# hongfz16/AvatarCLIP

Hardware: AMD Instinct MI355X
Metric: rays_per_sec_512x512_64spp_clip_guided_train_iter (higher is better)
Workload: dtype f16 (forward) / bf16 (gradient sweeps) MFMA operands, fp32 accumulate

## Files before the change

avatarclip_amd/csrc/avc_bwd_body.h:

```cpp
#pragma once
#include "avc_mlp.h"
constexpr int BWD_G = 4;
constexpr int BWD_WPB = 8;

template <typename P> __device__ __forceinline__ P launder(P p) {
  asm volatile("" : "+s"(p));
  return p;
}
__device__ __forceinline__ float second_term(float gbar_h, float g_a, float s) {
  const float r = s > 1e-30f ? __builtin_amdgcn_rcpf(s) : 0.f;
  return gbar_h * g_a * (AVC_BETA * (1.f - s) * r);
}
struct PF3 { h8 h0, h1; b8 b0, b1; h8 g0, g1; };

struct BwdArgs {
  PointSrc ps;
  long npts;
  const b8* Wb0;
  const float* T0;
  const float* d_sdf;
  const float* d_normal;
  const float* d_rgb;
  const float* rgb_fwd;
  const char* fpanels;
  char* gpanels;
  const unsigned short* masks;
  float* colsum;
};

#define AVC_CS_DUMMY 64
template <class N> struct ColSum {
  static constexpr int SLOT_FLOATS = PanelLayout<N>::CS_FLOATS + AVC_CS_DUMMY;
  static constexpr int LDS_BYTES = BWD_WPB * SLOT_FLOATS * 4;
};
typedef AVC_LDS float* cs_slot_t;
__device__ __forceinline__ float quad_xor1(float x) {
  return __builtin_bit_cast(float, __builtin_amdgcn_update_dpp(0, __builtin_bit_cast(int, x), 0xB1, 0xf, 0xf, true));
}
__device__ __forceinline__ float quad_xor2(float x) {
  return __builtin_bit_cast(float, __builtin_amdgcn_update_dpp(0, __builtin_bit_cast(int, x), 0x4E, 0xf, 0xf, true));
}
template <int NV>
__device__ __forceinline__ float transpose_sum(const float (&v)[NV], int lane) {
  static_assert(NV == 8 || NV == 16, "8 or 16 values per lane");
  float w[NV / 2];
  const bool b0 = lane & 1, b1 = lane & 2, b2 = lane & 4, b3 = lane & 8;
#pragma unroll
  for (int k = 0; k < NV / 2; ++k) w[k] = (b0 ? v[2 * k + 1] : v[2 * k]) + quad_xor1(b0 ? v[2 * k] : v[2 * k + 1]);
  float x[NV / 4];
#pragma unroll
  for (int k = 0; k < NV / 4; ++k) x[k] = (b1 ? w[2 * k + 1] : w[2 * k]) + quad_xor2(b1 ? w[2 * k] : w[2 * k + 1]);
  float y[NV / 8];
#pragma unroll
  for (int k = 0; k < NV / 8; ++k) y[k] = (b2 ? x[2 * k + 1] : x[2 * k]) + __shfl_xor(b2 ? x[2 * k] : x[2 * k + 1], 4);
  float z;
  if constexpr (NV == 16) z = (b3 ? y[1] : y[0]) + __shfl_xor(b3 ? y[0] : y[1], 8);
  else z = y[0] + __shfl_xor(y[0], 8);
  return z + __shfl_xor(z, 16);
}
template <class N, int NV>
__device__ __forceinline__ void col_sums(cs_slot_t slot, int lane, int base, const float (&v)[NV]) {
  const float total = transpose_sum<NV>(v, lane);
  const bool writer = (lane & 31) < NV;
  cs_slot_t dst = writer ? slot + base + (lane & (NV - 1)) : slot + PanelLayout<N>::CS_FLOATS + (lane & 63);
  *dst = *dst + total;
}
template <class N>
__device__ __forceinline__ cs_slot_t cs_init(char* lds_base, int wv, int lane) {
  cs_slot_t slot = (cs_slot_t)lds_base + wv * ColSum<N>::SLOT_FLOATS;
  for (int k = lane; k < ColSum<N>::SLOT_FLOATS; k += 64) slot[k] = 0.f;
  return slot;
}
template <class N>
__device__ __forceinline__ void cs_flush(cs_slot_t slot, float* out, long row, int lane) {
  asm volatile("s_waitcnt lgkmcnt(0)" ::: "memory");
  for (int k = lane; k < PanelLayout<N>::CS_FLOATS; k += 64) out[row * PanelLayout<N>::CS_FLOATS + k] = slot[k];
}

template <class N> struct BlkIn { b8 dof; unsigned m1[N::HT], m2[N::HT]; float dn[3], dsdf; };
template <class N>
__device__ __forceinline__ void load_blk_in(const BwdArgs& a, long blk, long nblk, int lane, BlkIn<N>& bi) {
  typedef PanelLayout<N> L;
  const int h = lane >> 5, p = lane & 31;
  long i = blk * 32 + p;
  const float vmask = i < a.npts ? 1.f : 0.f;
  if (i >= a.npts) i = a.npts - 1;
  bi.dof = zero_frag<b8>();
#pragma unroll
  for (int r = 0; r < 4; ++r) {
    const int ch = h ? 4 + r : r;
    const float c = (ch < 6) ? a.rgb_fwd[6 * i + (ch < 6 ? ch : 0)] : 0.f;
    const float dr = (ch < 6) ? a.d_rgb[6 * i + (ch < 6 ? ch : 0)] * vmask : 0.f;
    bi.dof[r] = (__bf16)(dr * c * (1.f - c));
  }
  const AVC_GLOBAL unsigned short* mk = as_global(a.masks) + (blk < nblk ? blk : nblk) * (long)L::MASK_U16 + lane;
#pragma unroll
  for (int t = 0; t < N::HT; ++t) {
    bi.m1[t] = mk[t * 64];
    bi.m2[t] = (N::NCMID == 1) ? mk[(N::HT + t) * 64] : 0u;
  }
#pragma unroll
  for (int c = 0; c < 3; ++c) bi.dn[c] = a.d_normal[3 * i + c] * vmask;
  bi.dsdf = a.d_sdf[i] * vmask;
}

template <class N>
__device__ __forceinline__ void bwd_sweeps(StageT<BWD_G>& sg, const BwdArgs& a, lds_tab_t Tl, long blk0, long nblk, int lane0,
                                           int wv, cs_slot_t cs, BlkIn<N>& bi, long blk0_next) {
  typedef PanelLayout<N> L;
  constexpr AvcOffsets o = Off<N>::value;
  const PointSrc& ps = a.ps;
  const long npts = a.npts;
  const b8* Wb = launder(a.Wb0);
  lds_tab_t T = Tl;
  asm volatile("" : "+s"(T));
  int lane = lane0;
  asm volatile("" : "+v"(lane));
  const int h = lane >> 5, p = lane & 31;
  sg.lane = lane;
  const long blk = blk0 + wv;
  const long bsel = blk < nblk ? blk : nblk;
  const PanelPtr ftiles = panel_ptr(const_cast<char*>(a.fpanels) + bsel * (long)L::P_TILES * 2048, lane);
  const PanelPtr tiles = panel_ptr(a.gpanels + bsel * (long)L::G_TILES * 2048, lane);
  long i = blk * 32 + p;
  const bool valid = i < npts;
  if (!valid) i = npts - 1;
  const float vmask = valid ? 1.f : 0.f;
  float x[3];
  fetch_point(ps, i, x);
  float nbar[3];
  float dsdf_in;
  {
    b8 dof[1];
    dof[0] = bi.dof;
    tile_store<false>(tiles, L::G_DO, dof[0], zero_frag<b8>());
    unsigned m1[N::HT], m2[N::HT];
#pragma unroll
    for (int t = 0; t < N::HT; ++t) { m1[t] = bi.m1[t]; m2[t] = bi.m2[t]; }
    const float dn_in[3] = {bi.dn[0], bi.dn[1], bi.dn[2]};
    dsdf_in = bi.dsdf;
#define AVC_RELU_BWD(OUT, MSK, PT)                                                                         \
  AVC_EPI(const unsigned bits = MSK[t];                                                                      \
          _Pragma("unroll") for (int j = 0; j < 8; ++j) {                                                    \
            OUT[2 * t][j] = (__bf16)(((bits >> relu_mask_bit(j)) & 1u) ? acc[j] : 0.f);                      \
            OUT[2 * t + 1][j] = (__bf16)(((bits >> relu_mask_bit(8 + j)) & 1u) ? acc[8 + j] : 0.f); }        \
          pin2(OUT[2 * t], OUT[2 * t + 1]);                                                                  \
          tile_store<false>(tiles, (PT) + t, OUT[2 * t], OUT[2 * t + 1]);)
    b8 dl[N::HK];
    b8 d1[N::HK];
    if constexpr (N::NCMID == 1) {
      layer_s1<b8, 1, N::HT>(sg, Wb, o.v[OFF_CHT], nxt<N, OFF_CM0T>(sg, Wb, o), dof, AVC_RELU_BWD(dl, m2, L::G_D2));
      layer_s1<b8, N::HK, N::HT>(sg, Wb, o.v[OFF_CM0T], nxt<N, OFF_C0T>(sg, Wb, o), dl, AVC_RELU_BWD(d1, m1, L::G_D1));
    } else {
      layer_s1<b8, 1, N::HT>(sg, Wb, o.v[OFF_CHT], nxt<N, OFF_C0T>(sg, Wb, o), dof, AVC_RELU_BWD(d1, m1, L::G_D1));
    }
    float dn_acc[3] = {0.f, 0.f, 0.f};
    layer_s1<b8, N::HK, N::HT + 1>(sg, Wb, o.v[OFF_C0T], nxt<N, OFF_W0G>(sg, Wb, o), d1, AVC_EPI(
      if (t < N::HT) {
        b8 f0, f1;
        _Pragma("unroll") for (int j = 0; j < 8; ++j) { f0[j] = (__bf16)acc[j]; f1[j] = (__bf16)acc[8 + j]; }
        pin2(f0, f1);
        tile_store<true>(tiles, L::G_DFEAT + (t < N::HT ? t : 0), f0, f1);
      } else {
        dn_acc[0] = acc[3]; dn_acc[1] = acc[0]; dn_acc[2] = acc[1];
      }
    ));
    {
      const float a3 = dn_acc[0], a0 = dn_acc[1], a1 = dn_acc[2];
      const float o3 = __shfl_xor(a3, 32), o0 = __shfl_xor(a0, 32), o1 = __shfl_xor(a1, 32);
      nbar[0] = valid ? dn_in[0] + (h ? o3 : a3) : 0.f;
      nbar[1] = valid ? dn_in[1] + (h ? a0 : o0) : 0.f;
      nbar[2] = valid ? dn_in[2] + (h ? a1 : o1) : 0.f;
    }
  }
  const float dsdf = dsdf_in;
  const float dsdfS = dsdf * AVC_S;
  {
    b8 fs = zero_frag<b8>();
    if (h == 0) {
      fs[0] = (__bf16)dsdf;
      fs[1] = (__bf16)(dsdf - (float)fs[0]);
    }
    tile_store<false>(tiles, L::G_SDF, fs, zero_frag<b8>());
  }
  b8 gbs[N::SK];
  b8 dfeat[N::HK];
  auto load_dfeat = [&]() __attribute__((always_inline)) {
#pragma unroll
    for (int t = 0; t < N::HT; ++t) {
      const FragPair<b8> d = tile_load<true, b8>(tiles, L::G_DFEAT + t);
      dfeat[2 * t] = d.a0;
      dfeat[2 * t + 1] = d.a1;
    }
  };
  {
    b8 gb0[3];
    {
      PE pe4;
      pe_compute(x, h, pe4);
      float g0[24];
#pragma unroll
      for (int q = 0; q < 24; ++q) {
        g0[q] = pe4.d[q] * nbar[q % 3];
        gb0[q >> 3][q & 7] = (__bf16)g0[q];
      }
#pragma unroll
      for (int s = 0; s < 3; ++s) {
        float v[8];
#pragma unroll
        for (int j = 0; j < 8; ++j) v[j] = g0[8 * s + j];
        col_sums<N, 8>(cs, lane, N::ST * 32 + (s * 2 + h) * 8, v);
      }
    }
    tile_store<false>(tiles, L::G_GB0, gb0[0], gb0[1]);
    tile_store<false>(tiles, L::G_GB0 + 1, gb0[2], zero_frag<b8>());
#define AVC_E_LOADH(PH) tile_load<false, h8>(ftiles, (PH) + t)
#define AVC_SECOND(OUT, PH, PT)                                                                              \
  AVC_PRE(return AVC_E_LOADH(PH);),                                                                          \
  AVC_EPID(FragPair<h8>, _Pragma("unroll") for (int j = 0; j < 8; ++j) {                                     \
            OUT[2 * t][j] = (__bf16)(acc[j] * sig_from_h((float)d.a0[j]));                                   \
            OUT[2 * t + 1][j] = (__bf16)(acc[8 + j] * sig_from_h((float)d.a1[j])); }                         \
          pin2(OUT[2 * t], OUT[2 * t + 1]);                                                                  \
          tile_store<true>(tiles, (PT) + t, OUT[2 * t], OUT[2 * t + 1]);)
#define AVC_SECOND_S(OUT, PH)                                                                                \
  AVC_PRE(return AVC_E_LOADH(PH);),                                                                          \
  AVC_EPID(FragPair<h8>, float v[16];                                                                        \
          _Pragma("unroll") for (int j = 0; j < 8; ++j) {                                                    \
            v[j] = acc[j] * sig_from_h((float)d.a0[j]);                                                      \
            v[8 + j] = acc[8 + j] * sig_from_h((float)d.a1[j]);                                              \
            OUT[2 * t][j] = (__bf16)v[j];                                                                    \
            OUT[2 * t + 1][j] = (__bf16)v[8 + j]; }                                                          \
          pin2(OUT[2 * t], OUT[2 * t + 1]);                                                                  \
          col_sums<N, 16>(cs, lane, (t * 2 + h) * 16, v);)
    b8 gb1[N::HK];
    layer_sq1<b8, 3, N::HT>(sg, Wb, o.v[OFF_W0G], nxt<N, OFF_WM0>(sg, Wb, o), gb0, AVC_SECOND(gb1, L::P_H1, L::G_GBH1));
    b8 gbm[N::HK];
    layer_sq1<b8, N::HK, N::HT>(sg, Wb, o.v[OFF_WM0], nxt<N, (N::NMID == 2 ? OFF_WM1 : OFF_WS)>(sg, Wb, o), gb1,
                                AVC_SECOND(gbm, L::P_HM, L::G_GBHM));
    b8 gbm1[N::HK];
    if constexpr (N::NMID == 2)
      layer_sq1<b8, N::HK, N::HT>(sg, Wb, o.v[OFF_WM1], nxt<N, OFF_WS>(sg, Wb, o), gbm,
                                  AVC_SECOND(gbm1, L::P_HM + N::HT, L::G_GBHM + N::HT));
    layer_sq1<b8, N::HK, N::ST>(sg, Wb, o.v[OFF_WS], nxt<N, OFF_WLT>(sg, Wb, o), (N::NMID == 2 ? gbm1 : gbm), AVC_SECOND_S(gbs, L::P_HS));
  }
  {
    b8 as_[N::SK];
    load_dfeat();
#define AVC_F_LOADB(PB) tile_load<true, b8>(tiles, (PB) + t)
#define AVC_LOAD3(PH, PB, PG)                                                                               \
  AVC_PRE(PF3 d; { const FragPair<h8> a_ = tile_load<true, h8>(ftiles, (PH) + t); d.h0 = a_.a0; d.h1 = a_.a1; } \
          { const FragPair<b8> a_ = AVC_F_LOADB(PB); d.b0 = a_.a0; d.b1 = a_.a1; } \
          { const FragPair<h8> a_ = tile_load<true, h8>(ftiles, (PG) + t); d.g0 = a_.a0; d.g1 = a_.a1; } return d;)
#define AVC_LOAD3_S(PH, PG)                                                                                 \
  AVC_PRE(PF3 d; { const FragPair<h8> a_ = tile_load<true, h8>(ftiles, (PH) + t); d.h0 = a_.a0; d.h1 = a_.a1; } \
          d.b0 = gbs[2 * t]; d.b1 = gbs[2 * t + 1];                                                          \
          { const FragPair<h8> a_ = tile_load<true, h8>(ftiles, (PG) + t); d.g0 = a_.a0; d.g1 = a_.a1; } return d;)
    layer_sq1<b8, N::HK, N::ST>(sg, Wb, o.v[OFF_WLT], nxt<N, OFF_WST>(sg, Wb, o), dfeat,
      AVC_LOAD3_S(L::P_HS, L::P_GAS), AVC_EPID(PF3,
      float wa[16];
      load16(T + o.v[OFF_WL0_ACC], t, h, wa);
      _Pragma("unroll") for (int j = 0; j < 8; ++j) {
        const float s0 = sig_from_h((float)d.h0[j]), s1 = sig_from_h((float)d.h1[j]);
        as_[2 * t][j] = (__bf16)(second_term((float)d.b0[j], (float)d.g0[j], s0) + (acc[j] + wa[j] * dsdfS) * s0);
        as_[2 * t + 1][j] = (__bf16)(second_term((float)d.b1[j], (float)d.g1[j], s1) + (acc[8 + j] + wa[8 + j] * dsdfS) * s1);
      }
      pin2(as_[2 * t], as_[2 * t + 1]);
      tile_store<false>(tiles, L::G_ABS + t, as_[2 * t], as_[2 * t + 1]);
    ));
#define AVC_REVERSE(OUT, PH, PB, PG, PT)                                                                    \
  AVC_LOAD3(PH, PB, PG),                                                                                     \
  AVC_EPID(PF3, _Pragma("unroll") for (int j = 0; j < 8; ++j) {                                              \
            const float s0 = sig_from_h((float)d.h0[j]), s1 = sig_from_h((float)d.h1[j]);                    \
            OUT[2 * t][j] = (__bf16)(second_term((float)d.b0[j], (float)d.g0[j], s0) + acc[j] * s0);         \
            OUT[2 * t + 1][j] = (__bf16)(second_term((float)d.b1[j], (float)d.g1[j], s1) + acc[8 + j] * s1); } \
          pin2(OUT[2 * t], OUT[2 * t + 1]);                                                                  \
          tile_store<false>(tiles, (PT) + t, OUT[2 * t], OUT[2 * t + 1]);)
    b8 am[N::HK];
    b8 am0[N::HK];
    const Next first = nxt<N, OFF_CHT>(sg, a.Wb0, o);
#define AVC_F_LASTHOOK AVC_HOOK(load_blk_in<N>(a, blk0_next + wv, nblk, lane, bi);)
    constexpr int TOP = (N::NMID - 1) * N::HT;
    layer_sq1<b8, N::SK, N::HT>(sg, Wb, o.v[OFF_WST], nxt<N, (N::NMID == 2 ? OFF_WM1T : OFF_WM0T)>(sg, Wb, o), as_,
                               AVC_REVERSE(am, L::P_HM + TOP, L::G_GBHM + TOP, L::P_GAM + TOP, L::G_ABM + TOP));
    if constexpr (N::NMID == 2)
      layer_sq1<b8, N::HK, N::HT>(sg, Wb, o.v[OFF_WM1T], nxt<N, OFF_WM0T>(sg, Wb, o), am,
                                 AVC_REVERSE(am0, L::P_HM, L::G_GBHM, L::P_GAM, L::G_ABM));
    layer_sq1<b8, N::HK, N::HT>(sg, Wb, o.v[OFF_WM0T], first, (N::NMID == 2 ? am0 : am),
                               AVC_REVERSE((N::NMID == 2 ? am : am0), L::P_H1, L::G_GBH1, L::P_GA1, L::G_AB1), AVC_F_LASTHOOK);
  }
#undef AVC_RELU_BWD
#undef AVC_SECOND
#undef AVC_LOAD3
#undef AVC_LOAD3_S
#undef AVC_F_LOADB
#undef AVC_E_LOADH
#undef AVC_SECOND_S
#undef AVC_F_LASTHOOK
#undef AVC_REVERSE
}
```

avatarclip_amd/csrc/avc_mlp.h:

```cpp
#pragma once
#include "avc_common.h"
#include "avc_stage.h"

template <int H_, int NMID_, int NCMID_>
struct NetT {
  static constexpr int H = H_;
  static constexpr int NMID = NMID_;
  static constexpr int NCMID = NCMID_;
  static constexpr int HT = H / 32;
  static constexpr int HK = H / 16;
  static constexpr int SKIP = H - 39;
  static constexpr int ST = (SKIP + 31) / 32;
  static constexpr int SK = 2 * ST;
  static_assert(H % 32 == 0 && SKIP > 0 && ST <= HT, "hidden width: a multiple of 32 above 39");
};
typedef NetT<256, 2, 1> NetFull;
typedef NetT<128, 1, 0> NetSmall;
typedef NetT<128, 2, 1> NetH128Deep;
typedef NetT<256, 1, 0> NetH256Shallow;
typedef NetT<64, 2, 1> NetH64Deep;
typedef NetT<64, 1, 0> NetH64Shallow;
template <class N> struct NetTag { typedef N type; };
template <typename R, typename F>
static inline R with_net(int net, R unknown, F&& f) {
  switch (net) {
    case 0: return f(NetTag<NetFull>{});
    case 1: return f(NetTag<NetSmall>{});
    case 2: return f(NetTag<NetH128Deep>{});
    case 3: return f(NetTag<NetH256Shallow>{});
    case 4: return f(NetTag<NetH64Deep>{});
    case 5: return f(NetTag<NetH64Shallow>{});
    default: return unknown;
  }
}
template <typename F>
static inline void for_each_net(F&& f) {
  for (int id = 0; with_net(id, false, [&](auto tag) { f(tag); return true; }); ++id) {}
}
#include "avc_offsets_gen.h"
template <class N> static inline bool offsets_match(const int* offs) {
  for (int k = 0; k < OFF_COUNT; ++k)
    if (offs[k] != Off<N>::value.v[k]) return false;
  return true;
}

struct PointSrc {
  const float* pts;
  const float* rays_o;
  const float* rays_d;
  const float* z;
  int S;
  int ldz;
  int midpoint;
  float sample_dist;
};

__device__ __forceinline__ void fetch_point(const PointSrc& ps, long i, float (&x)[3]) {
  if (ps.pts) {
    x[0] = ps.pts[3 * i]; x[1] = ps.pts[3 * i + 1]; x[2] = ps.pts[3 * i + 2];
    return;
  }
  const long ray = i / ps.S;
  const int s = (int)(i - ray * ps.S);
  const float* zr = ps.z + ray * ps.ldz;
  float t = zr[s];
  if (ps.midpoint) {
    const float dist = (s + 1 < ps.S) ? (zr[s + 1] - t) : ps.sample_dist;
    t = t + dist * 0.5f;
  }
#pragma unroll
  for (int c = 0; c < 3; ++c) x[c] = ps.rays_o[3 * ray + c] + ps.rays_d[3 * ray + c] * t;
}

template <typename V, int KS>
__device__ __forceinline__ const V* tptr(const V* blob, int off, int t, int lane) {
  return blob + (off >> 3) + (long)(t * KS) * 64 + lane;
}


template <class N, int OFF> struct TileInfo;
#define AVC_TI(OFF, KS_, NT_) template <class N> struct TileInfo<N, OFF> { static constexpr int KS = KS_, NT = NT_; };
AVC_TI(OFF_W0, 3, N::HT)          AVC_TI(OFF_WM0, N::HK, N::HT)   AVC_TI(OFF_WM1, N::HK, N::HT)  AVC_TI(OFF_WS, N::HK, N::ST)
AVC_TI(OFF_WL, N::SK + 3, N::HT)  AVC_TI(OFF_W0T, N::HK, 2)       AVC_TI(OFF_WM0T, N::HK, N::HT) AVC_TI(OFF_WM1T, N::HK, N::HT)
AVC_TI(OFF_WST, N::SK, N::HT)     AVC_TI(OFF_WLT, N::HK, N::ST)   AVC_TI(OFF_C0, N::HK + 1, N::HT) AVC_TI(OFF_CM0, N::HK, N::HT)
AVC_TI(OFF_CH, N::HK, 1)          AVC_TI(OFF_C0T, N::HK, N::HT + 1) AVC_TI(OFF_CM0T, N::HK, N::HT) AVC_TI(OFF_CHT, 1, N::HT)
AVC_TI(OFF_W0G, 3, N::HT)

template <class N, int OFF, class ST>
__device__ __forceinline__ Next nxt(const ST&, const void* blob, const AvcOffsets& o) {
  typedef TileInfo<N, OFF> TI;
  Next n;
  n.ptr = reinterpret_cast<const char*>(blob) + (long)o.v[OFF] * 2;
  constexpr int G = ST::template group<TI::KS>();
  static_assert(G >= 1 && G <= ST::G && TI::KS * 1024 * G <= ST::BUF_BYTES && TI::NT >= 1, "staging group of this layer");
  n.chunks = TI::KS * (TI::NT < G ? TI::NT : G);
  return n;
}
__device__ __forceinline__ Next no_next() { Next n; n.ptr = nullptr; n.chunks = 0; return n; }

#define AVC_SYNC() __syncthreads()
#define AVC_EPI(...) [&](int t, const facc& acc) __attribute__((always_inline)) { __VA_ARGS__ }
struct NoHook { __device__ __forceinline__ void operator()() const {} };
#define AVC_HOOK(...) [&]() __attribute__((always_inline)) { __VA_ARGS__ }
#define AVC_HOOKG(...) [&](int grp_, int ngrp_) __attribute__((always_inline)) { __VA_ARGS__ }
template <typename Hook>
__device__ __forceinline__ void hook_call(Hook&& hook, int g) {
  if constexpr (!std::is_invocable_v<Hook, int, int>) { if (g == 0) hook(); }
}
template <typename Hook>
__device__ __forceinline__ void hook_tile(Hook&& hook, int t, int nt) {
  if constexpr (std::is_invocable_v<Hook, int, int>) hook(t, nt);
}

#define AVC_PRE(...) [&](int t) __attribute__((always_inline)) { __VA_ARGS__ }
#define AVC_EPID(DT, ...) [&](int t, const facc& acc, const DT& d) __attribute__((always_inline)) { __VA_ARGS__ }
struct NoPre { __host__ __device__ __forceinline__ int operator()(int) const { return 0; } };
template <bool PAIRED, int KS, int NT, class ST, typename V, typename Mma, typename Pre, typename Epi, typename Hook>
__device__ __forceinline__ void layer_walk(ST& st, const V* __restrict__ blob, int offw, const Next& after, Mma&& mma, Pre&& pre,
                                           Epi&& epi, Hook&& hook) {
  constexpr int G = ST::template group<KS>();
  constexpr int NG = (NT + G - 1) / G;
  constexpr bool LOADS = !std::is_same_v<std::decay_t<Pre>, NoPre>;
  typedef std::invoke_result_t<Pre&, int> D;
  auto finish = [&](int t, const facc& acc, const D& d) __attribute__((always_inline)) {
    if constexpr (LOADS) epi(t, acc, d);
    else epi(t, acc);
  };
  facc prev0, prev1;
  D d0{}, d1{};
  int tp = -1, np = 0;
#pragma unroll
  for (int g = 0; g < NG; ++g) {
    AVC_SYNC();
    if (g + 1 < NG) {
      Next n;
      n.ptr = blob + (offw >> 3) + (long)((g + 1) * G * KS) * 64;
      n.chunks = KS * ((NT - (g + 1) * G) < G ? (NT - (g + 1) * G) : G);
      stage_issue(st, n, st.par ^ 1);
    } else {
      stage_issue(st, after, st.par ^ 1);
    }
    hook_call(hook, g);
#pragma unroll
    for (int j = 0; j < G; j += (PAIRED ? 2 : 1)) {
      const int t = g * G + j;
      if (t < NT) {
        const bool two = PAIRED && (j + 1 < G) && (t + 1 < NT);
        hook_tile(hook, t, NT);
        if (two) hook_tile(hook, t + 1, NT);
        if (LOADS && np > 0) {
          d0 = pre(tp);
          if (np > 1) d1 = pre(tp + 1);
          __builtin_amdgcn_sched_barrier(0);
        }
        facc a0, a1;
        mma(j, t, two, a0, a1);
        if (np > 0) {
          finish(tp, prev0, d0);
          if (np > 1) finish(tp + 1, prev1, d1);
          if (two) { interleave_mfma_valu<KS>(); interleave_mfma_valu<KS>(); } else interleave_mfma_valu<KS>();
        }
        prev0 = a0;
        if (two) prev1 = a1;
        tp = t; np = two ? 2 : 1;
        __builtin_amdgcn_sched_barrier(0);
      }
    }
    st.par ^= 1;
  }
  if constexpr (LOADS) {
    d0 = pre(tp);
    if (np > 1) d1 = pre(tp + 1);
  }
  finish(tp, prev0, d0);
  if (np > 1) finish(tp + 1, prev1, d1);
  __builtin_amdgcn_sched_barrier(0);
}
template <bool PAIRED, typename V, int KS, int NT, class ST, typename Pre, typename Epi, typename Hook, class Bias>
__device__ __forceinline__ void layer_sp(ST& st, const V* __restrict__ blob, int offw, const Next& after, const V (&in)[KS],
                                         Pre&& pre, Epi&& epi, Hook&& hook, const Bias& bias) {
  layer_walk<PAIRED, KS, NT>(st, blob, offw, after, [&](int j, int t, bool two, facc& a0, facc& a1) __attribute__((always_inline)) {
    if (two) tile_mma_pair<V, KS>(st, j, in, a0, a1, bias, t);
    else a0 = tile_mma<V, KS>(st, j, in, bias, t);
  }, pre, epi, hook);
}
template <typename V, int KS, int NT, class ST, typename Epi, typename Hook = NoHook, class Bias = NoBias>
__device__ __forceinline__ void layer_s(ST& st, const V* __restrict__ blob, int offw, const Next& after, const V (&in)[KS],
                                        Epi&& epi, Hook&& hook = NoHook{}, const Bias& bias = NoBias{}) {
  layer_sp<true, V, KS, NT>(st, blob, offw, after, in, NoPre{}, epi, hook, bias);
}
template <typename V, int KS, int NT, class ST, typename Epi, typename Hook = NoHook, class Bias = NoBias>
__device__ __forceinline__ void layer_s1(ST& st, const V* __restrict__ blob, int offw, const Next& after, const V (&in)[KS],
                                         Epi&& epi, Hook&& hook = NoHook{}, const Bias& bias = NoBias{}) {
  layer_sp<false, V, KS, NT>(st, blob, offw, after, in, NoPre{}, epi, hook, bias);
}
template <typename V, int KS, int NT, class ST, typename Pre, typename Epi, typename Hook = NoHook>
__device__ __forceinline__ void layer_sq(ST& st, const V* __restrict__ blob, int offw, const Next& after, const V (&in)[KS],
                                         Pre&& pre, Epi&& epi, Hook&& hook = NoHook{}) {
  layer_sp<true, V, KS, NT>(st, blob, offw, after, in, pre, epi, hook, NoBias{});
}
template <typename V, int KS, int NT, class ST, typename Pre, typename Epi, typename Hook = NoHook>
__device__ __forceinline__ void layer_sq1(ST& st, const V* __restrict__ blob, int offw, const Next& after, const V (&in)[KS],
                                          Pre&& pre, Epi&& epi, Hook&& hook = NoHook{}) {
  layer_sp<false, V, KS, NT>(st, blob, offw, after, in, pre, epi, hook, NoBias{});
}
template <typename V, int KA, int KB, int NT, class ST, typename Epi, typename Hook = NoHook, class Bias = NoBias>
__device__ __forceinline__ void layer2_s(ST& st, const V* __restrict__ blob, int offw, const Next& after, const V (&ina)[KA],
                                         const V (&inb)[KB], Epi&& epi, Hook&& hook = NoHook{}, const Bias& bias = NoBias{}) {
  layer_walk<true, KA + KB, NT>(st, blob, offw, after, [&](int j, int t, bool two, facc& a0, facc& a1) __attribute__((always_inline)) {
    if (two) tile_mma2_pair<V, KA, KB>(st, j, ina, inb, a0, a1, bias, t);
    else a0 = tile_mma2<V, KA, KB>(st, j, ina, inb, bias, t);
  }, NoPre{}, epi, hook);
}

template <class N>
struct PanelLayout {
  static constexpr int HT = N::HT, ST = N::ST, NM = N::NMID, NC = N::NCMID;
  static constexpr int P_H1 = 0;
  static constexpr int P_HM = P_H1 + HT;
  static constexpr int P_HS = P_HM + NM * HT;
  static constexpr int P_H0 = P_HS + ST;
  static constexpr int P_GA1 = P_H0 + 2;
  static constexpr int P_GAM = P_GA1 + HT;
  static constexpr int P_GAS = P_GAM + NM * HT;
  static constexpr int P_FEAT = P_GAS + ST;
  static constexpr int P_XN = P_FEAT + HT;
  static constexpr int P_R1 = P_XN + 1;
  static constexpr int P_R2 = P_R1 + HT;
  static constexpr int P_TILES = P_R2 + NC * HT;
  static constexpr int G_GBH1 = 0;
  static constexpr int G_GBHM = G_GBH1 + HT;
  static constexpr int G_GB0 = G_GBHM + NM * HT;
  static constexpr int G_AB1 = G_GB0 + 2;
  static constexpr int G_ABM = G_AB1 + HT;
  static constexpr int G_ABS = G_ABM + NM * HT;
  static constexpr int G_DFEAT = G_ABS + ST;
  static constexpr int G_SDF = G_DFEAT + HT;
  static constexpr int G_D1 = G_SDF + 1;
  static constexpr int G_D2 = G_D1 + HT;
  static constexpr int G_DO = G_D2 + NC * HT;
  static constexpr int G_TILES = G_DO + 1;
  static constexpr int MASK_U16 = 2 * HT * 64;
  static constexpr int CS_FLOATS = ST * 32 + 48;
};
template <class N>
struct ScratchLayout {
  static constexpr int HT = N::HT, NM = N::NMID;
  static constexpr int P_H1 = 0, P_HM = HT, P_FEAT = HT + NM * HT, P_TILES = P_FEAT + HT;
  static constexpr int P_H0 = 0, P_HS = 0, P_GA1 = 0, P_GAM = 0, P_GAS = 0, P_XN = 0, P_R1 = 0, P_R2 = 0;
};

struct PanelPtr {
  AVC_GLOBAL char* ub;
  unsigned off;
};
__device__ __forceinline__ PanelPtr panel_ptr(char* base, int lane) {
  const unsigned long long v = (unsigned long long)base;
  const unsigned lo = __builtin_amdgcn_readfirstlane((unsigned)v), hi = __builtin_amdgcn_readfirstlane((unsigned)(v >> 32));
  PanelPtr p;
  p.ub = (AVC_GLOBAL char*)(((unsigned long long)hi << 32) | lo);
  p.off = (unsigned)lane * 16u;
  return p;
}
template <typename V> __device__ __forceinline__ AVC_GLOBAL V* tile_addr(const PanelPtr& pp, int tile) {
  AVC_GLOBAL char* tb = pp.ub + (long)tile * 2048;
  asm("" : "+s"(tb));
  return (AVC_GLOBAL V*)(tb + pp.off);
}
template <typename V>
__device__ __forceinline__ V zero_frag() {
  V z;
#pragma unroll
  for (int j = 0; j < 8; ++j) z[j] = (typename MF<V>::S)0.f;
  return z;
}
template <bool KEEP, typename V>
__device__ __forceinline__ void tile_store(const PanelPtr& pp, int tile, const V& f0, const V& f1) {
  AVC_GLOBAL V* p = tile_addr<V>(pp, tile);
  if (KEEP) {
    p[0] = f0;
    p[64] = f1;
  } else {
    AVC_NT_STORE(f0, &p[0]);
    AVC_NT_STORE(f1, &p[64]);
  }
}
template <bool KEEP, int NT, typename V, int KS>
__device__ __forceinline__ void tiles_store(const PanelPtr& pp, int tile0, const V (&f)[KS]) {
#pragma unroll
  for (int t = 0; t < NT; ++t) tile_store<KEEP>(pp, tile0 + t, f[2 * t], f[2 * t + 1]);
}
template <bool KEEP, int NT, typename V, int KS>
__device__ __forceinline__ void tiles_store_part(const PanelPtr& pp, int tile0, const V (&f)[KS], int g, int ng) {
#pragma unroll
  for (int t = 0; t < NT; ++t)
    if (t * ng / NT == g) tile_store<KEEP>(pp, tile0 + t, f[2 * t], f[2 * t + 1]);
}
template <typename V> struct FragPair { V a0, a1; };
template <bool NT, typename V>
__device__ __forceinline__ FragPair<V> tile_load(const PanelPtr& pp, int tile) {
  const AVC_GLOBAL V* p = tile_addr<V>(pp, tile);
  FragPair<V> d;
  if (NT) { d.a0 = AVC_NT_LOAD(&p[0]); d.a1 = AVC_NT_LOAD(&p[64]); }
  else { d.a0 = p[0]; d.a1 = p[64]; }
  return d;
}

#define AVC_SDF_ACT(OUT)                                                                      \
  AVC_EPI(float a[16];                                                                        \
          softplus2_tile(acc, a);                                                             \
          acc_to_frags(a, OUT[2 * t], OUT[2 * t + 1]);)
template <class N, class ST, typename TP>
__device__ __forceinline__ float sdf_only(ST& sg, const h8* __restrict__ Wf, TP T, const AvcOffsets& o,
                                          int h, const float (&x)[3]) {
  PE pe;
  pe_compute(x, h, pe);
  float part = 0.f;
  {
    const auto wpe = T + o.v[OFF_WL0_PE] + h * 24;
#pragma unroll
    for (int q = 0; q < 24; ++q) part += wpe[q] * pe.v[q];
    asm volatile("" : "+v"(part));
  }
  h8 hlast[N::HK];
  {
    h8 h1[N::HK];
    {
      h8 pef[3];
      pe_to_frags_f16(pe, x, h, pef);
      layer_s1<h8, 3, N::HT>(sg, Wf, o.v[OFF_W0], nxt<N, OFF_WM0>(sg, Wf, o), pef, AVC_SDF_ACT(h1),
                             NoHook{}, TabBias{T + o.v[OFF_B0], h});
    }
    h8 hm0[N::HK];
    layer_s1<h8, N::HK, N::HT>(sg, Wf, o.v[OFF_WM0], nxt<N, (N::NMID == 2 ? OFF_WM1 : OFF_WS)>(sg, Wf, o), h1,
                               AVC_SDF_ACT((N::NMID == 2 ? hm0 : hlast)), NoHook{}, TabBias{T + o.v[OFF_BM0], h});
    if constexpr (N::NMID == 2)
      layer_s1<h8, N::HK, N::HT>(sg, Wf, o.v[OFF_WM1], nxt<N, OFF_WS>(sg, Wf, o), hm0, AVC_SDF_ACT(hlast),
                                 NoHook{}, TabBias{T + o.v[OFF_BM1], h});
  }
  layer_s1<h8, N::HK, N::ST>(sg, Wf, o.v[OFF_WS], no_next(), hlast, AVC_EPI(
    float w[16];
    load16(T + o.v[OFF_WL0_ACC], t, h, w);
    _Pragma("unroll") for (int r = 0; r < 16; ++r) part += w[r] * softplus2(acc[r]);
  ), NoHook{}, TabBias{T + o.v[OFF_BS], h});
  return xhalf_sum(part) + T[o.v[OFF_BL0]];
}
#undef AVC_SDF_ACT
```

avatarclip_amd/csrc/avc_mlp_bwd.hip:

```cpp
#include "avc_bwd_body.h"
#include "../../include/avc.h"

template <class N>
__global__ __launch_bounds__(64 * BWD_WPB) void mlp_bwd_kernel(BwdArgs a) {
  extern __shared__ __attribute__((aligned(16))) char lds[];
  typedef StageT<BWD_G> ST;
  constexpr AvcOffsets o = Off<N>::value;
  static_assert(BWD_WPB >= 4 && BWD_WPB % 4 == 0, "stage_issue's turns need a multiple of 4 wavefronts per workgroup");
  const int lane0 = threadIdx.x & 63;
  const int wv = threadIdx.x >> 6;
  const long nblk = (a.npts + 31) >> 5;
  ST sg = stage_init<BWD_G>(lds);
  stage_issue(sg, nxt<N, OFF_CHT>(sg, a.Wb0, o), 0);
  const lds_tab_t Tl = tab_to_lds(lds + ST::LDS_BYTES, a.T0, o.v[OFF_TAB_END]);
  const cs_slot_t cs = cs_init<N>(lds + ST::LDS_BYTES + AVC_TAB_LDS_BYTES, wv, lane0);
  __syncthreads();
  BlkIn<N> bi;
  load_blk_in<N>(a, (long)blockIdx.x * BWD_WPB + wv, nblk, lane0, bi);
  for (long blk0 = (long)blockIdx.x * BWD_WPB; blk0 < nblk; blk0 += (long)gridDim.x * BWD_WPB)
    bwd_sweeps<N>(sg, a, Tl, blk0, nblk, lane0, wv, cs, bi, blk0 + (long)gridDim.x * BWD_WPB);
  cs_flush<N>(cs, a.colsum, (long)blockIdx.x * BWD_WPB + wv, lane0);
}

extern "C" int avc_bwd_colsum_floats(int net) {
  return with_net<int>(net, 0, [](auto tag) -> int { return PanelLayout<typename decltype(tag)::type>::CS_FLOATS; });
}
extern "C" long avc_bwd_colsum_rows(long npts, long max_waves) {
  const long nblk = (npts + 31) / 32;
  long ngroups = (nblk + BWD_WPB - 1) / BWD_WPB, maxg = max_waves / BWD_WPB;
  if (maxg < 1) maxg = 1;
  long grid = ngroups < maxg ? ngroups : maxg;
  if (grid < 1) grid = 1;
  return grid * BWD_WPB;
}

extern "C" int avc_render_points_bwd(int net, const float* pts, const float* rays_o, const float* rays_d, const float* z,
                                     int S, int ldz, float sample_dist, long npts, const void* wbf16, const float* tab,
                                     const int* offs, const float* d_sdf, const float* d_normal, const float* d_rgb,
                                     const float* rgb_fwd, const void* fpanels, void* gpanels, const void* masks, float* colsum,
                                     long max_waves, void* stream) {
  if (npts <= 0) return 0;
  if (!fpanels || !gpanels || !masks || !rgb_fwd || !colsum) { avc_set_error("avc_render_points_bwd: fpanels / gpanels / masks / rgb_fwd / colsum == NULL"); return 1; }
  const int bad = with_net<int>(net, 2, [&](auto tag) -> int { return offsets_match<typename decltype(tag)::type>(offs) ? 0 : 1; });
  if (bad == 1) { avc_set_error("packed-blob offsets differ from the compiled-in table (regenerate csrc/avc_offsets_gen.h)"); return 1; }
  if (bad == 2) { avc_set_error("unknown net id"); return 1; }
  PointSrc ps{pts, rays_o, rays_d, z, S, ldz, pts ? 0 : 1, sample_dist};
  const long nblk = (npts + 31) / 32;
  long ngroups = (nblk + BWD_WPB - 1) / BWD_WPB;
  long maxg = max_waves / BWD_WPB;
  if (maxg < 1) maxg = 1;
  int grid = (int)(ngroups < maxg ? ngroups : maxg);
  if (grid < 1) grid = 1;
  hipStream_t s = (hipStream_t)stream;
  int cs_bytes = 0;
  for_each_net([&](auto tag) { const int b = ColSum<typename decltype(tag)::type>::LDS_BYTES; if (b > cs_bytes) cs_bytes = b; });
  const int lds_bytes = StageT<BWD_G>::LDS_BYTES + AVC_TAB_LDS_BYTES + cs_bytes;
  if (offs[OFF_TAB_END] * 4 > AVC_TAB_LDS_BYTES) { avc_set_error("fp32 table does not fit its LDS window"); return 1; }
  static unsigned long long attr_seen = 0;
  if (avc_first_use_on_device(attr_seen))
    for_each_net([&](auto tag) {
      (void)hipFuncSetAttribute((const void*)mlp_bwd_kernel<typename decltype(tag)::type>, hipFuncAttributeMaxDynamicSharedMemorySize, lds_bytes);
    });
  const BwdArgs args{ps, npts, (const b8*)wbf16, tab, d_sdf, d_normal, d_rgb, rgb_fwd, (const char*)fpanels, (char*)gpanels,
                     (const unsigned short*)masks, colsum};
  with_net<bool>(net, false, [&](auto tag) -> bool {
    hipLaunchKernelGGL((mlp_bwd_kernel<typename decltype(tag)::type>), dim3(grid), dim3(64 * BWD_WPB), lds_bytes, s, args);
    return true;
  });
  return avc_check_launch("avc_render_points_bwd");
}
```

avatarclip_amd/csrc/avc_mlp_fwd.hip:

```cpp
#include "avc_mlp.h"
constexpr int FWD_WPB = 8;
constexpr int SDF_WPB = 12;
constexpr int FWD_G = 4;
#define AVC_STORE_HOOK(KEEP, NT, PT, ARR) AVC_HOOKG(tiles_store_part<KEEP, NT>(tiles, PT, ARR, grp_, ngrp_);)
#include "../../include/avc.h"

template <class N>
__global__ __launch_bounds__(64 * SDF_WPB) void mlp_sdf_kernel(PointSrc ps, long npts, const h8* __restrict__ Wf,
                                                               const float* __restrict__ T,
                                                               float* __restrict__ sdf_out, const int* __restrict__ slot,
                                                               int ld_out) {
  constexpr AvcOffsets o = Off<N>::value;
  extern __shared__ __attribute__((aligned(16))) char lds[];
  typedef StageT<FWD_G> ST;
  static_assert(SDF_WPB >= 4 && SDF_WPB % 4 == 0, "stage_issue's turns need a multiple of 4 wavefronts per workgroup");
  const int lane = threadIdx.x & 63;
  const int h = lane >> 5;
  const int p = lane & 31;
  const long blk = (long)blockIdx.x * (blockDim.x >> 6) + (threadIdx.x >> 6);
  long i = blk * 32 + p;
  const bool valid = i < npts;
  if (!valid) i = npts - 1;
  ST sg = stage_init<ST::G>(lds);
  stage_issue(sg, nxt<N, OFF_W0>(sg, Wf, o), 0);
  const lds_tab_t Tl = tab_to_lds(lds + ST::LDS_BYTES, T, o.v[OFF_TAB_END]);
  __syncthreads();
  float x0[3];
  fetch_point(ps, i, x0);
  long oi = i;
  if (slot) {
    const long ray = i / ps.S;
    oi = ray * ld_out + slot[i];
  }
  const float sdfv = sdf_only<N>(sg, Wf, Tl, o, h, x0);
  if (valid && h == 0) sdf_out[oi] = sdfv;
}


template <typename P> __device__ __forceinline__ P launder_ptr(P p) {
  asm volatile("" : "+s"(p));
  return p;
}

template <class N, bool TRAIN>
__global__ __launch_bounds__(64 * FWD_WPB) void mlp_render_kernel(PointSrc ps, long npts, const h8* __restrict__ Wf0,
                                                                  const float* __restrict__ T0,
                                                                  float* __restrict__ sdf_out, float* __restrict__ normal_out,
                                                                  float* __restrict__ rgb_out, char* __restrict__ store,
                                                                  unsigned short* __restrict__ masks) {
  constexpr AvcOffsets o = Off<N>::value;
  typedef typename std::conditional<TRAIN, PanelLayout<N>, ScratchLayout<N>>::type L;
  extern __shared__ __attribute__((aligned(16))) char lds[];
  typedef StageT<FWD_G> ST;
  static_assert(FWD_WPB >= 4 && FWD_WPB % 4 == 0, "stage_issue's turns need a multiple of 4 wavefronts per workgroup");
  const int lane0 = threadIdx.x & 63;
  const int wv = threadIdx.x >> 6;
  const long nblk = (npts + 31) >> 5;
  const long wslot = (long)blockIdx.x * FWD_WPB + wv;
  char* slot0 = store + wslot * (long)L::P_TILES * 2048;
  ST sg = stage_init<FWD_G>(lds);
  stage_issue(sg, nxt<N, OFF_W0>(sg, Wf0, o), 0);
  const lds_tab_t Tl = tab_to_lds(lds + ST::LDS_BYTES, T0, o.v[OFF_TAB_END]);
  __syncthreads();
  for (long blk0 = (long)blockIdx.x * FWD_WPB; blk0 < nblk; blk0 += (long)gridDim.x * FWD_WPB) {
    const h8* Wf = launder_ptr(Wf0);
    lds_tab_t T = Tl;
    asm volatile("" : "+s"(T));
    int lane = lane0;
    asm volatile("" : "+v"(lane));
    const int h = lane >> 5, p = lane & 31;
    sg.lane = lane;
    const long blk = blk0 + wv;
    const PanelPtr tiles = panel_ptr(TRAIN ? store + (blk < nblk ? blk : nblk) * (long)L::P_TILES * 2048 : slot0, lane);
    AVC_GLOBAL unsigned short* mk = as_global(masks) + (TRAIN ? (blk < nblk ? blk : nblk) * (long)PanelLayout<N>::MASK_U16 + lane : 0);
    long i = blk * 32 + p;
    const bool valid = i < npts;
    if (!valid) i = npts - 1;
    float x[3];
    fetch_point(ps, i, x);
    float sdf;
    h8 g_s[N::SK];
    {
      h8 hs[N::SK];
      float part = 0.f;
      PE pe;
      pe_compute(x, h, pe);
      {
        const auto wpe = T + o.v[OFF_WL0_PE] + h * 24;
#pragma unroll
        for (int q = 0; q < 24; ++q) part += wpe[q] * pe.v[q];
        asm volatile("" : "+v"(part));
      }
      h8 pef[3];
      pe_to_frags_f16(pe, x, h, pef);
#define AVC_F_BIAS(OFFB) TabBias{T + o.v[OFFB], h}
#define AVC_F_ACT(OUT)                                                                        \
  AVC_EPI(float a[16];                                                                        \
          _Pragma("unroll") for (int r = 0; r < 16; ++r) a[r] = softplus2(acc[r]);           \
          acc_to_frags(a, OUT[2 * t], OUT[2 * t + 1]);)
#define AVC_F_LAST()                                                                          \
  AVC_EPI(float b[16], a[16];                                                                 \
          _Pragma("unroll") for (int r = 0; r < 16; ++r) a[r] = softplus2(acc[r]);           \
          load16(T + o.v[OFF_WL0_ACC], t, h, b);                                              \
          _Pragma("unroll") for (int r = 0; r < 16; ++r) part += b[r] * a[r];                 \
          acc_to_frags(a, hs[2 * t], hs[2 * t + 1]);                                          \
          float w0[8], w1[8];                                                                 \
          load8(T + o.v[OFF_WL0_FRAG], 2 * t, h, w0); load8(T + o.v[OFF_WL0_FRAG], 2 * t + 1, h, w1); \
          _Pragma("unroll") for (int j = 0; j < 8; ++j) {                                     \
            g_s[2 * t][j] = (_Float16)(w0[j] * sig_from_h(a[j]));                             \
            g_s[2 * t + 1][j] = (_Float16)(w1[j] * sig_from_h(a[8 + j])); }                   \
          pin2(g_s[2 * t], g_s[2 * t + 1]);)
      {
        h8 h1[N::HK];
        layer_s<h8, 3, N::HT>(sg, Wf, o.v[OFF_W0], nxt<N, OFF_WM0>(sg, Wf, o), pef, AVC_F_ACT(h1), AVC_HOOK(
          if constexpr (TRAIN) {
            tile_store<false>(tiles, L::P_H0, pef[0], pef[1]);
            tile_store<false>(tiles, L::P_H0 + 1, pef[2], zero_frag<h8>());
          }), AVC_F_BIAS(OFF_B0));
        h8 hm0[N::HK];
        layer_s<h8, N::HK, N::HT>(sg, Wf, o.v[OFF_WM0], nxt<N, (N::NMID == 2 ? OFF_WM1 : OFF_WS)>(sg, Wf, o), h1, AVC_F_ACT(hm0),
                                  AVC_STORE_HOOK(true, N::HT, L::P_H1, h1), AVC_F_BIAS(OFF_BM0));
        h8 hm1[N::HK];
        if constexpr (N::NMID == 2)
          layer_s<h8, N::HK, N::HT>(sg, Wf, o.v[OFF_WM1], nxt<N, OFF_WS>(sg, Wf, o), hm0, AVC_F_ACT(hm1),
                                    AVC_STORE_HOOK(true, N::HT, L::P_HM, hm0), AVC_F_BIAS(OFF_BM1));
        layer_s<h8, N::HK, N::ST>(sg, Wf, o.v[OFF_WS], nxt<N, OFF_WL>(sg, Wf, o), (N::NMID == 2 ? hm1 : hm0), AVC_F_LAST(),
                                  AVC_STORE_HOOK(true, N::HT, L::P_HM + (N::NMID - 1) * N::HT, (N::NMID == 2 ? hm1 : hm0)),
                                  AVC_F_BIAS(OFF_BS));
      }
      sdf = xhalf_sum(part) + T[o.v[OFF_BL0]];
      layer2_s<h8, N::SK, 3, N::HT>(sg, Wf, o.v[OFF_WL], nxt<N, OFF_WST>(sg, Wf, o), hs, pef, AVC_EPI(
        float a[16];
        _Pragma("unroll") for (int r = 0; r < 16; ++r) a[r] = acc[r];
        h8 f0, f1;
        acc_to_frags(a, f0, f1);
        tile_store<true>(tiles, L::P_FEAT + t, f0, f1);
      ), AVC_HOOK(
        if constexpr (TRAIN) {
          tiles_store<false, N::ST>(tiles, L::P_HS, hs);
          tiles_store<false, N::ST>(tiles, L::P_GAS, g_s);
        }), AVC_F_BIAS(OFF_BL));
    }
    float n[3];
    {
#define AVC_F_HLOAD(PH) tile_load<false, h8>(tiles, (PH) + t)
#define AVC_F_NSTEP(OUT, PH)                                                                              \
  AVC_PRE(return AVC_F_HLOAD(PH);),                                                                         \
  AVC_EPID(FragPair<h8>, _Pragma("unroll") for (int j = 0; j < 8; ++j) {                                    \
            OUT[2 * t][j] = (_Float16)(acc[j] * sig_from_h((float)d.a0[j]));                                \
            OUT[2 * t + 1][j] = (_Float16)(acc[8 + j] * sig_from_h((float)d.a1[j])); }                      \
          pin2(OUT[2 * t], OUT[2 * t + 1]);)
#define AVC_F_GSTORE(PG, G) AVC_HOOKG(if constexpr (TRAIN) tiles_store_part<false, N::HT>(tiles, PG, G, grp_, ngrp_);)
      h8 g[N::HK];
      h8 g2[N::HK];
      layer_sq<h8, N::SK, N::HT>(sg, Wf, o.v[OFF_WST], nxt<N, (N::NMID == 2 ? OFF_WM1T : OFF_WM0T)>(sg, Wf, o), g_s,
                                 AVC_F_NSTEP((N::NMID == 2 ? g : g2), L::P_HM + (N::NMID - 1) * N::HT));
      if constexpr (N::NMID == 2)
        layer_sq<h8, N::HK, N::HT>(sg, Wf, o.v[OFF_WM1T], nxt<N, OFF_WM0T>(sg, Wf, o), g, AVC_F_NSTEP(g2, L::P_HM),
                                   AVC_F_GSTORE(L::P_GAM + N::HT, g));
      layer_sq<h8, N::HK, N::HT>(sg, Wf, o.v[OFF_WM0T], nxt<N, OFF_W0T>(sg, Wf, o), g2, AVC_F_NSTEP(g, L::P_H1),
                                 AVC_F_GSTORE(L::P_GAM, g2));
      float part[3] = {0.f, 0.f, 0.f};
      const auto wpe = T + o.v[OFF_WL0_PE] + h * 24;
      float x2[3] = {x[0], x[1], x[2]};
      asm volatile("" : "+v"(x2[0]), "+v"(x2[1]), "+v"(x2[2]));
      PE pe2;
      pe_compute(x2, h, pe2);
      layer_s<h8, N::HK, 2>(sg, Wf, o.v[OFF_W0T], nxt<N, OFF_C0>(sg, Wf, o), g, AVC_EPI(
        _Pragma("unroll") for (int r = 0; r < 16; ++r) {
          const int q = 16 * t + r;
          if (q < 24) part[q % 3] += pe2.d[q] * (acc[r] + wpe[q]);
        }
      ), AVC_F_GSTORE(L::P_GA1, g));
#pragma unroll
      for (int c = 0; c < 3; ++c) n[c] = xhalf_sum(part[c]);
    }
    float rgb[4];
    {
      h8 xn[1];
#pragma unroll
      for (int j = 0; j < 8; ++j) xn[0][j] = (_Float16)0.f;
      if (h == 0) {
#pragma unroll
        for (int c = 0; c < 3; ++c) { xn[0][c] = (_Float16)x[c]; xn[0][3 + c] = (_Float16)n[c]; }
      }
      h8 feat[N::HK];
#pragma unroll
      for (int t = 0; t < N::HT; ++t) {
        const FragPair<h8> d = tile_load<false, h8>(tiles, L::P_FEAT + t);
        feat[2 * t] = d.a0;
        feat[2 * t + 1] = d.a1;
      }
#define AVC_F_RELU(OUT, ML)                                                                   \
  AVC_EPI(const unsigned bits = relu_frags<TRAIN>(acc, OUT[2 * t], OUT[2 * t + 1]);            \
          if constexpr (TRAIN) mk[((ML) * N::HT + t) * 64] = (unsigned short)bits;)
#define AVC_F_RSTORE(PT, R)                                                                   \
  AVC_HOOKG(if constexpr (TRAIN) tiles_store_part<false, N::HT>(tiles, PT, R, grp_, ngrp_);)
      h8 r1[N::HK];
      layer2_s<h8, N::HK, 1, N::HT>(sg, Wf, o.v[OFF_C0], nxt<N, (N::NCMID == 1 ? OFF_CM0 : OFF_CH)>(sg, Wf, o), feat, xn, AVC_F_RELU(r1, 0),
        AVC_HOOK(if constexpr (TRAIN) tile_store<false>(tiles, L::P_XN, xn[0], zero_frag<h8>());), AVC_F_BIAS(OFF_CB0));
      h8 r2[N::HK];
      if constexpr (N::NCMID == 1)
        layer_s<h8, N::HK, N::HT>(sg, Wf, o.v[OFF_CM0], nxt<N, OFF_CH>(sg, Wf, o), r1, AVC_F_RELU(r2, 1),
                                  AVC_F_RSTORE(L::P_R1, r1), AVC_F_BIAS(OFF_CBM0));
      layer_s<h8, N::HK, 1>(sg, Wf, o.v[OFF_CH], nxt<N, OFF_W0>(sg, Wf0, o), (N::NCMID == 1 ? r2 : r1), AVC_EPI(
        float b[16];
        load16(T + o.v[OFF_CBH], 0, h, b);
        _Pragma("unroll") for (int r = 0; r < 4; ++r) rgb[r] = sigmoidf_(acc[r] + b[r]);
      ), AVC_F_RSTORE((N::NCMID == 1 ? L::P_R2 : L::P_R1), (N::NCMID == 1 ? r2 : r1)));
    }
    if (valid) {
      if (h == 0) {
        sdf_out[i] = sdf;
        normal_out[3 * i + 0] = n[0]; normal_out[3 * i + 1] = n[1]; normal_out[3 * i + 2] = n[2];
        rgb_out[6 * i + 0] = rgb[0]; rgb_out[6 * i + 1] = rgb[1]; rgb_out[6 * i + 2] = rgb[2]; rgb_out[6 * i + 3] = rgb[3];
      } else {
        rgb_out[6 * i + 4] = rgb[0]; rgb_out[6 * i + 5] = rgb[1];
      }
    }
  }
}

#define AVC_NET_CONST(R, EXPR) with_net<R>(net, 0, [](auto tag) -> R { typedef typename decltype(tag)::type N; return EXPR; })
extern "C" long avc_fwd_scratch_bytes_per_wave(int net) { return AVC_NET_CONST(long, (long)ScratchLayout<N>::P_TILES * 2048); }
extern "C" int avc_fwd_panel_tiles(int net) { return AVC_NET_CONST(int, PanelLayout<N>::P_TILES); }
extern "C" int avc_grad_panel_tiles(int net) { return AVC_NET_CONST(int, PanelLayout<N>::G_TILES); }
extern "C" int avc_mask_u16_per_block(int net) { return AVC_NET_CONST(int, PanelLayout<N>::MASK_U16); }
#undef AVC_NET_CONST

static int grid_for(long npts, int waves_per_block, int max_blocks) {
  long nblk = (npts + 31) / 32;
  long g = (nblk + waves_per_block - 1) / waves_per_block;
  if (g > max_blocks) g = max_blocks;
  if (g < 1) g = 1;
  return (int)g;
}

static int check_tab(const int* offs) {
  if (offs[OFF_TAB_END] * 4 > AVC_TAB_LDS_BYTES) { avc_set_error("fp32 table does not fit its LDS window"); return 1; }
  return 0;
}
static int check_offsets(int net, const int* offs) {
  const int r = with_net<int>(net, 2, [&](auto tag) -> int { return offsets_match<typename decltype(tag)::type>(offs) ? 0 : 1; });
  if (r == 1) avc_set_error("packed-blob offsets differ from the compiled-in table (regenerate csrc/avc_offsets_gen.h)");
  if (r == 2) avc_set_error("unknown net id");
  return r;
}

static int launch_sdf(int net, PointSrc ps, long npts, const void* wf, const float* tab, const int* offs,
                      float* sdf_out, const int* slot, int ld_out, void* stream) {
  if (npts <= 0) return 0;
  if (check_tab(offs)) return 1;
  if (check_offsets(net, offs)) return 1;
  hipStream_t s = (hipStream_t)stream;
  const int lds_bytes = StageT<FWD_G>::LDS_BYTES + AVC_TAB_LDS_BYTES;
  static unsigned long long attr_seen = 0;
  if (avc_first_use_on_device(attr_seen))
    for_each_net([&](auto tag) {
      (void)hipFuncSetAttribute((const void*)mlp_sdf_kernel<typename decltype(tag)::type>, hipFuncAttributeMaxDynamicSharedMemorySize, lds_bytes);
    });
  const int wpb = SDF_WPB;
  const int grid = grid_for(npts, wpb, 0x7fffffff);
  const bool known = with_net<bool>(net, false, [&](auto tag) -> bool {
    hipLaunchKernelGGL((mlp_sdf_kernel<typename decltype(tag)::type>), dim3(grid), dim3(64 * wpb), lds_bytes, s, ps, npts, (const h8*)wf, tab,
                       sdf_out, slot, ld_out);
    return true;
  });
  if (!known) { avc_set_error("unknown net id"); return 1; }
  return avc_check_launch("avc_sdf_forward");
}

extern "C" int avc_sdf_forward(int net, const float* pts, const float* rays_o, const float* rays_d, const float* z,
                               int S, int ldz, long npts, const void* wf16, const float* tab, const int* offs,
                               float* sdf_out, const int* slot, int ld_out, void* stream) {
  PointSrc ps{pts, rays_o, rays_d, z, S, ldz, 0, 0.f};
  return launch_sdf(net, ps, npts, wf16, tab, offs, sdf_out, slot, ld_out, stream);
}

template <bool TRAIN>
static int launch_render(int net, PointSrc ps, long npts, const void* wf16, const float* tab, const int* offs, float* sdf_out,
                         float* normal_out, float* rgb_out, long max_waves, void* store, void* masks, void* stream,
                         const char* what) {
  if (check_tab(offs)) return 1;
  if (check_offsets(net, offs)) return 1;
  long maxg = max_waves / FWD_WPB;
  if (maxg < 1) maxg = 1;
  const int grid = grid_for(npts, FWD_WPB, (int)(maxg < 0x7fffffff ? maxg : 0x7fffffff));
  const int lds_bytes = StageT<FWD_G>::LDS_BYTES + AVC_TAB_LDS_BYTES;
  hipStream_t s = (hipStream_t)stream;
  static unsigned long long attr_seen = 0;
  if (avc_first_use_on_device(attr_seen))
    for_each_net([&](auto tag) {
      (void)hipFuncSetAttribute((const void*)mlp_render_kernel<typename decltype(tag)::type, TRAIN>, hipFuncAttributeMaxDynamicSharedMemorySize, lds_bytes);
    });
  const bool known = with_net<bool>(net, false, [&](auto tag) -> bool {
    hipLaunchKernelGGL((mlp_render_kernel<typename decltype(tag)::type, TRAIN>), dim3(grid), dim3(64 * FWD_WPB), lds_bytes, s, ps, npts, (const h8*)wf16, tab,
                       sdf_out, normal_out, rgb_out, (char*)store, (unsigned short*)masks);
    return true;
  });
  if (!known) { avc_set_error("unknown net id"); return 1; }
  return avc_check_launch(what);
}

extern "C" int avc_render_points_fwd(int net, const float* pts, const float* rays_o, const float* rays_d,
                                     const float* z, int S, int ldz, float sample_dist, long npts, const void* wf16,
                                     const float* tab, const int* offs, float* sdf_out, float* normal_out,
                                     float* rgb_out, long max_waves, void* scratch, void* stream) {
  if (npts <= 0) return 0;
  if (!scratch) { avc_set_error("avc_render_points_fwd: scratch == NULL"); return 1; }
  PointSrc ps{pts, rays_o, rays_d, z, S, ldz, pts ? 0 : 1, sample_dist};
  return launch_render<false>(net, ps, npts, wf16, tab, offs, sdf_out, normal_out, rgb_out, max_waves, scratch, nullptr, stream,
                              "avc_render_points_fwd");
}

extern "C" int avc_render_points_fwd_train(int net, const float* pts, const float* rays_o, const float* rays_d,
                                           const float* z, int S, int ldz, float sample_dist, long npts, const void* wf16,
                                           const float* tab, const int* offs, float* sdf_out, float* normal_out,
                                           float* rgb_out, long max_waves, void* panels, void* masks, void* stream) {
  if (npts <= 0) return 0;
  if (!panels || !masks) { avc_set_error("avc_render_points_fwd_train: panels / masks == NULL"); return 1; }
  PointSrc ps{pts, rays_o, rays_d, z, S, ldz, pts ? 0 : 1, sample_dist};
  return launch_render<true>(net, ps, npts, wf16, tab, offs, sdf_out, normal_out, rgb_out, max_waves, panels, masks, stream,
                             "avc_render_points_fwd_train");
}
```

avatarclip_amd/csrc/avc_stage.h:

```cpp
#pragma once
#include "avc_common.h"

#define STAGE_TILE_BYTES (16 * 1024)

struct Next {
  const void* ptr;
  int chunks;
};

template <int G_>
struct StageT {
  static constexpr int G = G_;
  static constexpr int BUF_BYTES = G_ * STAGE_TILE_BYTES;
  static constexpr int LDS_BYTES = 2 * G_ * STAGE_TILE_BYTES;
  template <int KS> static constexpr int group() { return (KS * 1024 * G_ <= BUF_BYTES) ? G_ : BUF_BYTES / (KS * 1024); }
  char* lds;
  int par;
  int wave;
  int lane;
  int nw;
  int turn;
};

template <int G>
__device__ __forceinline__ StageT<G> stage_init(char* lds) {
  StageT<G> st;
  st.lds = lds;
  st.par = 0;
  st.wave = __builtin_amdgcn_readfirstlane((int)(threadIdx.x >> 6));
  st.lane = threadIdx.x & 63;
  st.nw = blockDim.x >> 6;
  st.turn = 0;
  return st;
}

template <class ST>
__device__ __forceinline__ void stage_issue(ST& st, const Next& nx, int buf, bool rotate = true) {
  if (!nx.ptr) return;
  const char* g = reinterpret_cast<const char*>(nx.ptr);
  char* dst = st.lds + buf * ST::BUF_BYTES;
  int first = st.wave, stride = st.nw;
  if (rotate) {
    const int nsub = st.nw >> 2;
    first = ((st.wave >> 2) == st.turn) ? (st.wave & 3) : nx.chunks;
    stride = 4;
    const int nt = st.turn + 1;
    st.turn = nt >= nsub ? 0 : nt;
  }
  for (int c = first; c < nx.chunks; c += stride)
    __builtin_amdgcn_global_load_lds((const __attribute__((address_space(1))) void*)(g + c * 1024 + st.lane * 16),
                                     (__attribute__((address_space(3))) void*)(dst + c * 1024), 16, 0, 0);
}


template <typename V>
__device__ __forceinline__ void pin4(V& a, V& b, V& c, V& d) { asm("" : "+v"(a), "+v"(b), "+v"(c), "+v"(d)); }

constexpr int AVC_VALU_PER_MFMA = 10;
template <int KS>
__device__ __forceinline__ void interleave_mfma_valu() {
#pragma unroll
  for (int k = 0; k < KS; ++k) {
    __builtin_amdgcn_sched_group_barrier(0x008, 1, 0);
    __builtin_amdgcn_sched_group_barrier(0x002, AVC_VALU_PER_MFMA, 0);
  }
}
constexpr int AVC_LDS_AHEAD = 8;
template <typename V, int KS>
__device__ __forceinline__ facc mma_chain_lds(const V* __restrict__ a_lds , const V (&in)[KS], facc acc) {
  V a[KS];
#pragma unroll
  for (int s = 0; s < KS && s < AVC_LDS_AHEAD; ++s) a[s] = a_lds[s * 64];
#pragma unroll
  for (int s = 0; s < KS; s += 4) {
    if (s + 3 < KS) pin4(a[s], a[s + 1], a[s + 2], a[s + 3]);
#pragma unroll
    for (int k = s + AVC_LDS_AHEAD; k < s + AVC_LDS_AHEAD + 4 && k < KS; ++k) a[k] = a_lds[k * 64];
#pragma unroll
    for (int k = s; k < s + 4 && k < KS; ++k) acc = MF<V>::mma(a[k], in[k], acc);
  }
  return acc;
}


struct NoBias { static constexpr bool on = false; };
struct TabBias { static constexpr bool on = true; lds_tab_t tab; int h; };

constexpr int AVC_LDS_AHEAD2 = 4;
template <typename V, int KS>
__device__ __forceinline__ void pair_chain(const V* __restrict__ a0, const V* __restrict__ a1, const V (&in)[KS], facc& acc0, facc& acc1) {
  V fa[KS], fb[KS];
#pragma unroll
  for (int s = 0; s < KS && s < AVC_LDS_AHEAD2; ++s) { fa[s] = a0[s * 64]; fb[s] = a1[s * 64]; }
#pragma unroll
  for (int s = 0; s < KS; s += 2) {
    if (s + 1 < KS) pin4(fa[s], fb[s], fa[s + 1], fb[s + 1]);
#pragma unroll
    for (int k = s + AVC_LDS_AHEAD2; k < s + AVC_LDS_AHEAD2 + 2 && k < KS; ++k) { fa[k] = a0[k * 64]; fb[k] = a1[k * 64]; }
#pragma unroll
    for (int k = s; k < s + 2 && k < KS; ++k) {
      acc0 = MF<V>::mma(fa[k], in[k], acc0);
      acc1 = MF<V>::mma(fb[k], in[k], acc1);
    }
  }
}
template <class B>
__device__ __forceinline__ void pair_init(facc& acc0, facc& acc1, const B& bias, int t) {
  if constexpr (B::on) {
    float b0[16], b1[16];
    load16(bias.tab, t, bias.h, b0);
    load16(bias.tab, t + 1, bias.h, b1);
#pragma unroll
    for (int r = 0; r < 16; ++r) { acc0[r] = b0[r]; acc1[r] = b1[r]; }
  } else {
#pragma unroll
    for (int r = 0; r < 16; ++r) { acc0[r] = 0.f; acc1[r] = 0.f; }
  }
}
template <typename V, int KS, class ST, class B>
__device__ __forceinline__ void tile_mma_pair(const ST& st, int j, const V (&in)[KS], facc& acc0, facc& acc1, const B& bias, int t) {
  const V* a0 = reinterpret_cast<const V*>(st.lds + st.par * ST::BUF_BYTES + j * KS * 1024) + st.lane;
  pair_init(acc0, acc1, bias, t);
  pair_chain<V, KS>(a0, a0 + KS * 64, in, acc0, acc1);
}
template <typename V, int KA, int KB, class ST, class B>
__device__ __forceinline__ void tile_mma2_pair(const ST& st, int j, const V (&ina)[KA], const V (&inb)[KB], facc& acc0, facc& acc1,
                                               const B& bias, int t) {
  const V* a0 = reinterpret_cast<const V*>(st.lds + st.par * ST::BUF_BYTES + j * (KA + KB) * 1024) + st.lane;
  const V* a1 = a0 + (KA + KB) * 64;
  pair_init(acc0, acc1, bias, t);
  pair_chain<V, KA>(a0, a1, ina, acc0, acc1);
  pair_chain<V, KB>(a0 + KA * 64, a1 + KA * 64, inb, acc0, acc1);
}

template <class B>
__device__ __forceinline__ facc acc_init(const B& bias, int t) {
  facc acc;
  if constexpr (B::on) {
    float b[16];
    load16(bias.tab, t, bias.h, b);
#pragma unroll
    for (int r = 0; r < 16; ++r) acc[r] = b[r];
  } else {
#pragma unroll
    for (int r = 0; r < 16; ++r) acc[r] = 0.f;
  }
  return acc;
}
template <typename V, int KS, class ST, class B = NoBias>
__device__ __forceinline__ facc tile_mma(const ST& st, int j, const V (&in)[KS], const B& bias = NoBias{}, int t = 0) {
  const facc acc = acc_init(bias, t);
  const V* a = reinterpret_cast<const V*>(st.lds + st.par * ST::BUF_BYTES + j * KS * 1024) + st.lane;
  return mma_chain_lds<V, KS>(a, in, acc);
}
template <typename V, int KA, int KB, class ST, class B = NoBias>
__device__ __forceinline__ facc tile_mma2(const ST& st, int j, const V (&ina)[KA], const V (&inb)[KB], const B& bias = NoBias{}, int t = 0) {
  facc acc = acc_init(bias, t);
  const V* a = reinterpret_cast<const V*>(st.lds + st.par * ST::BUF_BYTES + j * (KA + KB) * 1024) + st.lane;
  acc = mma_chain_lds<V, KA>(a, ina, acc);
  return mma_chain_lds<V, KB>(a + KA * 64, inb, acc);
}
```

Baseline: 2.453 million.

## Add vmcnt-counted stage sync infrastructure and inline-asm LDS weight staging

```diff
diff --git a/avatarclip_amd/csrc/avc_bwd_body.h b/avatarclip_amd/csrc/avc_bwd_body.h
--- a/avatarclip_amd/csrc/avc_bwd_body.h
+++ b/avatarclip_amd/csrc/avc_bwd_body.h
@@ -1,6 +1,7 @@
 #pragma once
 #include "avc_mlp.h"
 constexpr int BWD_G = 4;
+typedef StageT<BWD_G, false> BwdStage;
 constexpr int BWD_WPB = 8;
 
 template <typename P> __device__ __forceinline__ P launder(P p) {
@@ -11,7 +12,7 @@
   const float r = s > 1e-30f ? __builtin_amdgcn_rcpf(s) : 0.f;
   return gbar_h * g_a * (AVC_BETA * (1.f - s) * r);
 }
-struct PF3 { h8 h0, h1; b8 b0, b1; h8 g0, g1; };
+template <int NLOADS> struct PF3T { h8 h0, h1; b8 b0, b1; h8 g0, g1; static constexpr int vm = NLOADS; };
 
 struct BwdArgs {
   PointSrc ps;
@@ -105,12 +106,13 @@
 }
 
 template <class N>
-__device__ __forceinline__ void bwd_sweeps(StageT<BWD_G>& sg, const BwdArgs& a, lds_tab_t Tl, long blk0, long nblk, int lane0,
+__device__ __forceinline__ void bwd_sweeps(BwdStage& sg, const BwdArgs& a, lds_tab_t Tl, long blk0, long nblk, int lane0,
                                            int wv, cs_slot_t cs, BlkIn<N>& bi, long blk0_next) {
   typedef PanelLayout<N> L;
   constexpr AvcOffsets o = Off<N>::value;
   const PointSrc& ps = a.ps;
   const long npts = a.npts;
+  stage_block_top(sg);
   const b8* Wb = launder(a.Wb0);
   lds_tab_t T = Tl;
   asm volatile("" : "+s"(T));
@@ -145,7 +147,7 @@
             OUT[2 * t][j] = (__bf16)(((bits >> relu_mask_bit(j)) & 1u) ? acc[j] : 0.f);                      \
             OUT[2 * t + 1][j] = (__bf16)(((bits >> relu_mask_bit(8 + j)) & 1u) ? acc[8 + j] : 0.f); }        \
           pin2(OUT[2 * t], OUT[2 * t + 1]);                                                                  \
-          tile_store<false>(tiles, (PT) + t, OUT[2 * t], OUT[2 * t + 1]);)
+          vm_ += tile_store<false>(tiles, (PT) + t, OUT[2 * t], OUT[2 * t + 1]);)
     b8 dl[N::HK];
     b8 d1[N::HK];
     if constexpr (N::NCMID == 1) {
@@ -160,7 +162,7 @@
         b8 f0, f1;
         _Pragma("unroll") for (int j = 0; j < 8; ++j) { f0[j] = (__bf16)acc[j]; f1[j] = (__bf16)acc[8 + j]; }
         pin2(f0, f1);
-        tile_store<true>(tiles, L::G_DFEAT + (t < N::HT ? t : 0), f0, f1);
+        vm_ += tile_store<true>(tiles, L::G_DFEAT + (t < N::HT ? t : 0), f0, f1);
       } else {
         dn_acc[0] = acc[3]; dn_acc[1] = acc[0]; dn_acc[2] = acc[1];
       }
@@ -221,7 +223,7 @@
             OUT[2 * t][j] = (__bf16)(acc[j] * sig_from_h((float)d.a0[j]));                                   \
             OUT[2 * t + 1][j] = (__bf16)(acc[8 + j] * sig_from_h((float)d.a1[j])); }                         \
           pin2(OUT[2 * t], OUT[2 * t + 1]);                                                                  \
-          tile_store<true>(tiles, (PT) + t, OUT[2 * t], OUT[2 * t + 1]);)
+          vm_ += tile_store<true>(tiles, (PT) + t, OUT[2 * t], OUT[2 * t + 1]);)
 #define AVC_SECOND_S(OUT, PH)                                                                                \
   AVC_PRE(return AVC_E_LOADH(PH);),                                                                          \
   AVC_EPID(FragPair<h8>, float v[16];                                                                        \
@@ -248,15 +250,15 @@
     load_dfeat();
 #define AVC_F_LOADB(PB) tile_load<true, b8>(tiles, (PB) + t)
 #define AVC_LOAD3(PH, PB, PG)                                                                               \
-  AVC_PRE(PF3 d; { const FragPair<h8> a_ = tile_load<true, h8>(ftiles, (PH) + t); d.h0 = a_.a0; d.h1 = a_.a1; } \
+  AVC_PRE(PF3T<6> d; { const FragPair<h8> a_ = tile_load<true, h8>(ftiles, (PH) + t); d.h0 = a_.a0; d.h1 = a_.a1; } \
           { const FragPair<b8> a_ = AVC_F_LOADB(PB); d.b0 = a_.a0; d.b1 = a_.a1; } \
           { const FragPair<h8> a_ = tile_load<true, h8>(ftiles, (PG) + t); d.g0 = a_.a0; d.g1 = a_.a1; } return d;)
 #define AVC_LOAD3_S(PH, PG)                                                                                 \
-  AVC_PRE(PF3 d; { const FragPair<h8> a_ = tile_load<true, h8>(ftiles, (PH) + t); d.h0 = a_.a0; d.h1 = a_.a1; } \
+  AVC_PRE(PF3T<4> d; { const FragPair<h8> a_ = tile_load<true, h8>(ftiles, (PH) + t); d.h0 = a_.a0; d.h1 = a_.a1; } \
           d.b0 = gbs[2 * t]; d.b1 = gbs[2 * t + 1];                                                          \
           { const FragPair<h8> a_ = tile_load<true, h8>(ftiles, (PG) + t); d.g0 = a_.a0; d.g1 = a_.a1; } return d;)
     layer_sq1<b8, N::HK, N::ST>(sg, Wb, o.v[OFF_WLT], nxt<N, OFF_WST>(sg, Wb, o), dfeat,
-      AVC_LOAD3_S(L::P_HS, L::P_GAS), AVC_EPID(PF3,
+      AVC_LOAD3_S(L::P_HS, L::P_GAS), AVC_EPID(PF3T<4>,
       float wa[16];
       load16(T + o.v[OFF_WL0_ACC], t, h, wa);
       _Pragma("unroll") for (int j = 0; j < 8; ++j) {
@@ -265,16 +267,16 @@
         as_[2 * t + 1][j] = (__bf16)(second_term((float)d.b1[j], (float)d.g1[j], s1) + (acc[8 + j] + wa[8 + j] * dsdfS) * s1);
       }
       pin2(as_[2 * t], as_[2 * t + 1]);
-      tile_store<false>(tiles, L::G_ABS + t, as_[2 * t], as_[2 * t + 1]);
+      vm_ += tile_store<false>(tiles, L::G_ABS + t, as_[2 * t], as_[2 * t + 1]);
     ));
 #define AVC_REVERSE(OUT, PH, PB, PG, PT)                                                                    \
   AVC_LOAD3(PH, PB, PG),                                                                                     \
-  AVC_EPID(PF3, _Pragma("unroll") for (int j = 0; j < 8; ++j) {                                              \
+  AVC_EPID(PF3T<6>, _Pragma("unroll") for (int j = 0; j < 8; ++j) {                                          \
             const float s0 = sig_from_h((float)d.h0[j]), s1 = sig_from_h((float)d.h1[j]);                    \
             OUT[2 * t][j] = (__bf16)(second_term((float)d.b0[j], (float)d.g0[j], s0) + acc[j] * s0);         \
             OUT[2 * t + 1][j] = (__bf16)(second_term((float)d.b1[j], (float)d.g1[j], s1) + acc[8 + j] * s1); } \
           pin2(OUT[2 * t], OUT[2 * t + 1]);                                                                  \
-          tile_store<false>(tiles, (PT) + t, OUT[2 * t], OUT[2 * t + 1]);)
+          vm_ += tile_store<false>(tiles, (PT) + t, OUT[2 * t], OUT[2 * t + 1]);)
     b8 am[N::HK];
     b8 am0[N::HK];
     const Next first = nxt<N, OFF_CHT>(sg, a.Wb0, o);
diff --git a/avatarclip_amd/csrc/avc_mlp.h b/avatarclip_amd/csrc/avc_mlp.h
--- a/avatarclip_amd/csrc/avc_mlp.h
+++ b/avatarclip_amd/csrc/avc_mlp.h
@@ -98,22 +98,28 @@
 }
 __device__ __forceinline__ Next no_next() { Next n; n.ptr = nullptr; n.chunks = 0; return n; }
 
-#define AVC_SYNC() __syncthreads()
-#define AVC_EPI(...) [&](int t, const facc& acc) __attribute__((always_inline)) { __VA_ARGS__ }
-struct NoHook { __device__ __forceinline__ void operator()() const {} };
-#define AVC_HOOK(...) [&]() __attribute__((always_inline)) { __VA_ARGS__ }
-#define AVC_HOOKG(...) [&](int grp_, int ngrp_) __attribute__((always_inline)) { __VA_ARGS__ }
+#define AVC_SYNC(st) stage_sync(st)
+#define AVC_EPI(...) [&](int t, const facc& acc) __attribute__((always_inline)) { int vm_ = 0; __VA_ARGS__ return vm_; }
+struct NoHook { __device__ __forceinline__ int operator()() const { return 0; } };
+#define AVC_HOOK(...) [&]() __attribute__((always_inline)) { int vm_ = 0; __VA_ARGS__ return vm_; }
+#define AVC_HOOKG(...) [&](int grp_, int ngrp_) __attribute__((always_inline)) { int vm_ = 0; __VA_ARGS__ return vm_; }
 template <typename Hook>
-__device__ __forceinline__ void hook_call(Hook&& hook, int g) {
-  if constexpr (!std::is_invocable_v<Hook, int, int>) { if (g == 0) hook(); }
+__device__ __forceinline__ int hook_call(Hook&& hook, int g) {
+  if constexpr (!std::is_invocable_v<Hook, int, int>) { if (g == 0) return hook(); }
+  return 0;
 }
 template <typename Hook>
-__device__ __forceinline__ void hook_tile(Hook&& hook, int t, int nt) {
-  if constexpr (std::is_invocable_v<Hook, int, int>) hook(t, nt);
+__device__ __forceinline__ int hook_tile(Hook&& hook, int t, int nt) {
+  if constexpr (std::is_invocable_v<Hook, int, int>) return hook(t, nt);
+  return 0;
+}
+template <class D> constexpr int loads_vm() {
+  if constexpr (std::is_class_v<D>) return D::vm;
+  else return 0;
 }
 
 #define AVC_PRE(...) [&](int t) __attribute__((always_inline)) { __VA_ARGS__ }
-#define AVC_EPID(DT, ...) [&](int t, const facc& acc, const DT& d) __attribute__((always_inline)) { __VA_ARGS__ }
+#define AVC_EPID(DT, ...) [&](int t, const facc& acc, const DT& d) __attribute__((always_inline)) { int vm_ = 0; __VA_ARGS__ return vm_; }
 struct NoPre { __host__ __device__ __forceinline__ int operator()(int) const { return 0; } };
 template <bool PAIRED, int KS, int NT, class ST, typename V, typename Mma, typename Pre, typename Epi, typename Hook>
 __device__ __forceinline__ void layer_walk(ST& st, const V* __restrict__ blob, int offw, const Next& after, Mma&& mma, Pre&& pre,
@@ -123,15 +129,15 @@
   constexpr bool LOADS = !std::is_same_v<std::decay_t<Pre>, NoPre>;
   typedef std::invoke_result_t<Pre&, int> D;
   auto finish = [&](int t, const facc& acc, const D& d) __attribute__((always_inline)) {
-    if constexpr (LOADS) epi(t, acc, d);
-    else epi(t, acc);
+    if constexpr (LOADS) return epi(t, acc, d);
+    else return epi(t, acc);
   };
   facc prev0, prev1;
   D d0{}, d1{};
   int tp = -1, np = 0;
 #pragma unroll
   for (int g = 0; g < NG; ++g) {
-    AVC_SYNC();
+    AVC_SYNC(st);
     if (g + 1 < NG) {
       Next n;
       n.ptr = blob + (offw >> 3) + (long)((g + 1) * G * KS) * 64;
@@ -140,24 +146,25 @@
     } else {
       stage_issue(st, after, st.par ^ 1);
     }
-    hook_call(hook, g);
+    st.vm += hook_call(hook, g);
 #pragma unroll
     for (int j = 0; j < G; j += (PAIRED ? 2 : 1)) {
       const int t = g * G + j;
       if (t < NT) {
         const bool two = PAIRED && (j + 1 < G) && (t + 1 < NT);
-        hook_tile(hook, t, NT);
-        if (two) hook_tile(hook, t + 1, NT);
         if (LOADS && np > 0) {
           d0 = pre(tp);
           if (np > 1) d1 = pre(tp + 1);
-          __builtin_amdgcn_sched_barrier(0);
+          st.vm += np * loads_vm<D>();
         }
+        st.vm += hook_tile(hook, t, NT);
+        if (two) st.vm += hook_tile(hook, t + 1, NT);
+        if (LOADS && np > 0) __builtin_amdgcn_sched_barrier(0);
         facc a0, a1;
         mma(j, t, two, a0, a1);
         if (np > 0) {
-          finish(tp, prev0, d0);
-          if (np > 1) finish(tp + 1, prev1, d1);
+          st.vm += finish(tp, prev0, d0);
+          if (np > 1) st.vm += finish(tp + 1, prev1, d1);
           if (two) { interleave_mfma_valu<KS>(); interleave_mfma_valu<KS>(); } else interleave_mfma_valu<KS>();
         }
         prev0 = a0;
@@ -171,9 +178,10 @@
   if constexpr (LOADS) {
     d0 = pre(tp);
     if (np > 1) d1 = pre(tp + 1);
-  }
-  finish(tp, prev0, d0);
-  if (np > 1) finish(tp + 1, prev1, d1);
+    st.vm += np * loads_vm<D>();
+  }
+  st.vm += finish(tp, prev0, d0);
+  if (np > 1) st.vm += finish(tp + 1, prev1, d1);
   __builtin_amdgcn_sched_barrier(0);
 }
 template <bool PAIRED, typename V, int KS, int NT, class ST, typename Pre, typename Epi, typename Hook, class Bias>
@@ -275,7 +283,7 @@
   return z;
 }
 template <bool KEEP, typename V>
-__device__ __forceinline__ void tile_store(const PanelPtr& pp, int tile, const V& f0, const V& f1) {
+__device__ __forceinline__ int tile_store(const PanelPtr& pp, int tile, const V& f0, const V& f1) {
   AVC_GLOBAL V* p = tile_addr<V>(pp, tile);
   if (KEEP) {
     p[0] = f0;
@@ -284,19 +292,24 @@
     AVC_NT_STORE(f0, &p[0]);
     AVC_NT_STORE(f1, &p[64]);
   }
+  return 2;
 }
 template <bool KEEP, int NT, typename V, int KS>
-__device__ __forceinline__ void tiles_store(const PanelPtr& pp, int tile0, const V (&f)[KS]) {
-#pragma unroll
-  for (int t = 0; t < NT; ++t) tile_store<KEEP>(pp, tile0 + t, f[2 * t], f[2 * t + 1]);
+__device__ __forceinline__ int tiles_store(const PanelPtr& pp, int tile0, const V (&f)[KS]) {
+  int vm = 0;
+#pragma unroll
+  for (int t = 0; t < NT; ++t) vm += tile_store<KEEP>(pp, tile0 + t, f[2 * t], f[2 * t + 1]);
+  return vm;
 }
 template <bool KEEP, int NT, typename V, int KS>
-__device__ __forceinline__ void tiles_store_part(const PanelPtr& pp, int tile0, const V (&f)[KS], int g, int ng) {
+__device__ __forceinline__ int tiles_store_part(const PanelPtr& pp, int tile0, const V (&f)[KS], int g, int ng) {
+  int vm = 0;
 #pragma unroll
   for (int t = 0; t < NT; ++t)
-    if (t * ng / NT == g) tile_store<KEEP>(pp, tile0 + t, f[2 * t], f[2 * t + 1]);
-}
-template <typename V> struct FragPair { V a0, a1; };
+    if (t * ng / NT == g) vm += tile_store<KEEP>(pp, tile0 + t, f[2 * t], f[2 * t + 1]);
+  return vm;
+}
+template <typename V> struct FragPair { V a0, a1; static constexpr int vm = 2; };
 template <bool NT, typename V>
 __device__ __forceinline__ FragPair<V> tile_load(const PanelPtr& pp, int tile) {
   const AVC_GLOBAL V* p = tile_addr<V>(pp, tile);
diff --git a/avatarclip_amd/csrc/avc_mlp_bwd.hip b/avatarclip_amd/csrc/avc_mlp_bwd.hip
--- a/avatarclip_amd/csrc/avc_mlp_bwd.hip
+++ b/avatarclip_amd/csrc/avc_mlp_bwd.hip
@@ -4,17 +4,17 @@
 template <class N>
 __global__ __launch_bounds__(64 * BWD_WPB) void mlp_bwd_kernel(BwdArgs a) {
   extern __shared__ __attribute__((aligned(16))) char lds[];
-  typedef StageT<BWD_G> ST;
+  typedef BwdStage ST;
   constexpr AvcOffsets o = Off<N>::value;
   static_assert(BWD_WPB >= 4 && BWD_WPB % 4 == 0, "stage_issue's turns need a multiple of 4 wavefronts per workgroup");
   const int lane0 = threadIdx.x & 63;
   const int wv = threadIdx.x >> 6;
   const long nblk = (a.npts + 31) >> 5;
-  ST sg = stage_init<BWD_G>(lds);
+  ST sg = stage_init<ST>(lds);
   stage_issue(sg, nxt<N, OFF_CHT>(sg, a.Wb0, o), 0);
   const lds_tab_t Tl = tab_to_lds(lds + ST::LDS_BYTES, a.T0, o.v[OFF_TAB_END]);
   const cs_slot_t cs = cs_init<N>(lds + ST::LDS_BYTES + AVC_TAB_LDS_BYTES, wv, lane0);
-  __syncthreads();
+  stage_barrier_lds();
   BlkIn<N> bi;
   load_blk_in<N>(a, (long)blockIdx.x * BWD_WPB + wv, nblk, lane0, bi);
   for (long blk0 = (long)blockIdx.x * BWD_WPB; blk0 < nblk; blk0 += (long)gridDim.x * BWD_WPB)
@@ -54,7 +54,7 @@
   hipStream_t s = (hipStream_t)stream;
   int cs_bytes = 0;
   for_each_net([&](auto tag) { const int b = ColSum<typename decltype(tag)::type>::LDS_BYTES; if (b > cs_bytes) cs_bytes = b; });
-  const int lds_bytes = StageT<BWD_G>::LDS_BYTES + AVC_TAB_LDS_BYTES + cs_bytes;
+  const int lds_bytes = BwdStage::LDS_BYTES + AVC_TAB_LDS_BYTES + cs_bytes;
   if (offs[OFF_TAB_END] * 4 > AVC_TAB_LDS_BYTES) { avc_set_error("fp32 table does not fit its LDS window"); return 1; }
   static unsigned long long attr_seen = 0;
   if (avc_first_use_on_device(attr_seen))
diff --git a/avatarclip_amd/csrc/avc_mlp_fwd.hip b/avatarclip_amd/csrc/avc_mlp_fwd.hip
--- a/avatarclip_amd/csrc/avc_mlp_fwd.hip
+++ b/avatarclip_amd/csrc/avc_mlp_fwd.hip
@@ -2,7 +2,7 @@
 constexpr int FWD_WPB = 8;
 constexpr int SDF_WPB = 12;
 constexpr int FWD_G = 4;
-#define AVC_STORE_HOOK(KEEP, NT, PT, ARR) AVC_HOOKG(tiles_store_part<KEEP, NT>(tiles, PT, ARR, grp_, ngrp_);)
+#define AVC_STORE_HOOK(KEEP, NT, PT, ARR) AVC_HOOKG(vm_ += tiles_store_part<KEEP, NT>(tiles, PT, ARR, grp_, ngrp_);)
 #include "../../include/avc.h"
 
 template <class N>
@@ -12,7 +12,7 @@
                                                                int ld_out) {
   constexpr AvcOffsets o = Off<N>::value;
   extern __shared__ __attribute__((aligned(16))) char lds[];
-  typedef StageT<FWD_G> ST;
+  typedef StageT<FWD_G, false> ST;
   static_assert(SDF_WPB >= 4 && SDF_WPB % 4 == 0, "stage_issue's turns need a multiple of 4 wavefronts per workgroup");
   const int lane = threadIdx.x & 63;
   const int h = lane >> 5;
@@ -21,10 +21,10 @@
   long i = blk * 32 + p;
   const bool valid = i < npts;
   if (!valid) i = npts - 1;
-  ST sg = stage_init<ST::G>(lds);
+  ST sg = stage_init<ST>(lds);
   stage_issue(sg, nxt<N, OFF_W0>(sg, Wf, o), 0);
   const lds_tab_t Tl = tab_to_lds(lds + ST::LDS_BYTES, T, o.v[OFF_TAB_END]);
-  __syncthreads();
+  stage_barrier_lds();
   float x0[3];
   fetch_point(ps, i, x0);
   long oi = i;
@@ -58,11 +58,12 @@
   const long nblk = (npts + 31) >> 5;
   const long wslot = (long)blockIdx.x * FWD_WPB + wv;
   char* slot0 = store + wslot * (long)L::P_TILES * 2048;
-  ST sg = stage_init<FWD_G>(lds);
+  ST sg = stage_init<ST>(lds);
   stage_issue(sg, nxt<N, OFF_W0>(sg, Wf0, o), 0);
   const lds_tab_t Tl = tab_to_lds(lds + ST::LDS_BYTES, T0, o.v[OFF_TAB_END]);
-  __syncthreads();
+  stage_barrier_lds();
   for (long blk0 = (long)blockIdx.x * FWD_WPB; blk0 < nblk; blk0 += (long)gridDim.x * FWD_WPB) {
+    stage_block_top(sg);
     const h8* Wf = launder_ptr(Wf0);
     lds_tab_t T = Tl;
     asm volatile("" : "+s"(T));
@@ -114,8 +115,8 @@
         h8 h1[N::HK];
         layer_s<h8, 3, N::HT>(sg, Wf, o.v[OFF_W0], nxt<N, OFF_WM0>(sg, Wf, o), pef, AVC_F_ACT(h1), AVC_HOOK(
           if constexpr (TRAIN) {
-            tile_store<false>(tiles, L::P_H0, pef[0], pef[1]);
-            tile_store<false>(tiles, L::P_H0 + 1, pef[2], zero_frag<h8>());
+            vm_ += tile_store<false>(tiles, L::P_H0, pef[0], pef[1]);
+            vm_ += tile_store<false>(tiles, L::P_H0 + 1, pef[2], zero_frag<h8>());
           }), AVC_F_BIAS(OFF_B0));
         h8 hm0[N::HK];
         layer_s<h8, N::HK, N::HT>(sg, Wf, o.v[OFF_WM0], nxt<N, (N::NMID == 2 ? OFF_WM1 : OFF_WS)>(sg, Wf, o), h1, AVC_F_ACT(hm0),
@@ -134,11 +135,11 @@
         _Pragma("unroll") for (int r = 0; r < 16; ++r) a[r] = acc[r];
         h8 f0, f1;
         acc_to_frags(a, f0, f1);
-        tile_store<true>(tiles, L::P_FEAT + t, f0, f1);
+        vm_ += tile_store<true>(tiles, L::P_FEAT + t, f0, f1);
       ), AVC_HOOK(
         if constexpr (TRAIN) {
-          tiles_store<false, N::ST>(tiles, L::P_HS, hs);
-          tiles_store<false, N::ST>(tiles, L::P_GAS, g_s);
+          vm_ += tiles_store<false, N::ST>(tiles, L::P_HS, hs);
+          vm_ += tiles_store<false, N::ST>(tiles, L::P_GAS, g_s);
         }), AVC_F_BIAS(OFF_BL));
     }
     float n[3];
@@ -150,7 +151,7 @@
             OUT[2 * t][j] = (_Float16)(acc[j] * sig_from_h((float)d.a0[j]));                                \
             OUT[2 * t + 1][j] = (_Float16)(acc[8 + j] * sig_from_h((float)d.a1[j])); }                      \
           pin2(OUT[2 * t], OUT[2 * t + 1]);)
-#define AVC_F_GSTORE(PG, G) AVC_HOOKG(if constexpr (TRAIN) tiles_store_part<false, N::HT>(tiles, PG, G, grp_, ngrp_);)
+#define AVC_F_GSTORE(PG, G) AVC_HOOKG(if constexpr (TRAIN) vm_ += tiles_store_part<false, N::HT>(tiles, PG, G, grp_, ngrp_);)
       h8 g[N::HK];
       h8 g2[N::HK];
       layer_sq<h8, N::SK, N::HT>(sg, Wf, o.v[OFF_WST], nxt<N, (N::NMID == 2 ? OFF_WM1T : OFF_WM0T)>(sg, Wf, o), g_s,
@@ -193,12 +194,12 @@
       }
 #define AVC_F_RELU(OUT, ML)                                                                   \
   AVC_EPI(const unsigned bits = relu_frags<TRAIN>(acc, OUT[2 * t], OUT[2 * t + 1]);            \
-          if constexpr (TRAIN) mk[((ML) * N::HT + t) * 64] = (unsigned short)bits;)
+          if constexpr (TRAIN) { mk[((ML) * N::HT + t) * 64] = (unsigned short)bits; vm_ += 1; })
 #define AVC_F_RSTORE(PT, R)                                                                   \
-  AVC_HOOKG(if constexpr (TRAIN) tiles_store_part<false, N::HT>(tiles, PT, R, grp_, ngrp_);)
+  AVC_HOOKG(if constexpr (TRAIN) vm_ += tiles_store_part<false, N::HT>(tiles, PT, R, grp_, ngrp_);)
       h8 r1[N::HK];
       layer2_s<h8, N::HK, 1, N::HT>(sg, Wf, o.v[OFF_C0], nxt<N, (N::NCMID == 1 ? OFF_CM0 : OFF_CH)>(sg, Wf, o), feat, xn, AVC_F_RELU(r1, 0),
-        AVC_HOOK(if constexpr (TRAIN) tile_store<false>(tiles, L::P_XN, xn[0], zero_frag<h8>());), AVC_F_BIAS(OFF_CB0));
+        AVC_HOOK(if constexpr (TRAIN) vm_ += tile_store<false>(tiles, L::P_XN, xn[0], zero_frag<h8>());), AVC_F_BIAS(OFF_CB0));
       h8 r2[N::HK];
       if constexpr (N::NCMID == 1)
         layer_s<h8, N::HK, N::HT>(sg, Wf, o.v[OFF_CM0], nxt<N, OFF_CH>(sg, Wf, o), r1, AVC_F_RELU(r2, 1),
diff --git a/avatarclip_amd/csrc/avc_stage.h b/avatarclip_amd/csrc/avc_stage.h
--- a/avatarclip_amd/csrc/avc_stage.h
+++ b/avatarclip_amd/csrc/avc_stage.h
@@ -8,9 +8,10 @@
   int chunks;
 };
 
-template <int G_>
+template <int G_, bool COUNTED_ = true>
 struct StageT {
   static constexpr int G = G_;
+  static constexpr bool COUNTED = COUNTED_;
   static constexpr int BUF_BYTES = G_ * STAGE_TILE_BYTES;
   static constexpr int LDS_BYTES = 2 * G_ * STAGE_TILE_BYTES;
   template <int KS> static constexpr int group() { return (KS * 1024 * G_ <= BUF_BYTES) ? G_ : BUF_BYTES / (KS * 1024); }
@@ -20,17 +21,21 @@
   int lane;
   int nw;
   int turn;
+  bool mine;
+  int vm;
 };
 
-template <int G>
-__device__ __forceinline__ StageT<G> stage_init(char* lds) {
-  StageT<G> st;
+template <class ST>
+__device__ __forceinline__ ST stage_init(char* lds) {
+  ST st;
   st.lds = lds;
   st.par = 0;
   st.wave = __builtin_amdgcn_readfirstlane((int)(threadIdx.x >> 6));
   st.lane = threadIdx.x & 63;
   st.nw = blockDim.x >> 6;
   st.turn = 0;
+  st.mine = false;
+  st.vm = 0;
   return st;
 }
 
@@ -38,7 +43,7 @@
 __device__ __forceinline__ void stage_issue(ST& st, const Next& nx, int buf, bool rotate = true) {
   if (!nx.ptr) return;
   const char* g = reinterpret_cast<const char*>(nx.ptr);
-  char* dst = st.lds + buf * ST::BUF_BYTES;
+  const unsigned dst = (unsigned)(unsigned long long)(AVC_LDS char*)(st.lds + buf * ST::BUF_BYTES);
   int first = st.wave, stride = st.nw;
   if (rotate) {
     const int nsub = st.nw >> 2;
@@ -47,11 +52,41 @@
     const int nt = st.turn + 1;
     st.turn = nt >= nsub ? 0 : nt;
   }
-  for (int c = first; c < nx.chunks; c += stride)
-    __builtin_amdgcn_global_load_lds((const __attribute__((address_space(1))) void*)(g + c * 1024 + st.lane * 16),
-                                     (__attribute__((address_space(3))) void*)(dst + c * 1024), 16, 0, 0);
+  st.mine = first < nx.chunks;
+  st.vm = 0;
+  for (int c = first; c < nx.chunks; c += stride) {
+    const AVC_GLOBAL char* src = (const AVC_GLOBAL char*)(g + c * 1024 + st.lane * 16);
+    const unsigned d = __builtin_amdgcn_readfirstlane(dst + c * 1024);
+    unsigned keep;
+    asm volatile("s_mov_b32 %0, m0\n\ts_mov_b32 m0, %2\n\ts_nop 0\n\tglobal_load_lds_dwordx4 %1, off\n\ts_mov_b32 m0, %0"
+                 : "=&s"(keep) : "v"(src), "s"(d) : "memory");
+  }
 }
 
+__device__ __forceinline__ void stage_wait_vmcnt(int n) {
+  switch (n) {
+#define ST_W(k) case k: asm volatile("s_waitcnt vmcnt(%0)" ::"n"(k) : "memory"); break;
+#define ST_W8(k) ST_W(k) ST_W(k + 1) ST_W(k + 2) ST_W(k + 3) ST_W(k + 4) ST_W(k + 5) ST_W(k + 6) ST_W(k + 7)
+    ST_W8(0) ST_W8(8) ST_W8(16) ST_W8(24) ST_W8(32) ST_W8(40) ST_W8(48) ST_W8(56)
+#undef ST_W8
+#undef ST_W
+    default: asm volatile("s_waitcnt vmcnt(0)" ::: "memory"); break;
+  }
+}
+constexpr int STAGE_VMCNT_MAX = 63;
+template <class ST>
+__device__ __forceinline__ void stage_sync(ST& st) {
+  if constexpr (ST::COUNTED) {
+    if (st.mine) stage_wait_vmcnt(st.vm < STAGE_VMCNT_MAX ? st.vm : STAGE_VMCNT_MAX);
+  } else {
+    stage_wait_vmcnt(0);
+  }
+  st.mine = false;
+  asm volatile("s_waitcnt lgkmcnt(0)\n\ts_barrier" ::: "memory");
+}
+__device__ __forceinline__ void stage_barrier_lds() { asm volatile("s_waitcnt lgkmcnt(0)\n\ts_barrier" ::: "memory"); }
+template <class ST>
+__device__ __forceinline__ void stage_block_top(ST& st) { st.vm = 0; }
 
 template <typename V>
 __device__ __forceinline__ void pin4(V& a, V& b, V& c, V& d) { asm("" : "+v"(a), "+v"(b), "+v"(c), "+v"(d)); }
```

Result: no change. 2.457 million (median of 6 runs) (+0.2%).
